# sabarim/STEm-Seg

Measured on AMD Instinct MI355X. Metric: clips/sec (T=8, 480p) embed+cluster, higher is better.
Workload: dtype f16x3: fp32 emulated from 2 fp16 terms per operand (22-bit operand significands; fp32 has 24), power-of-two operand scaling, 3 fp16 MFMA products per fp32 product, fp32 accumulate; |activation| >= 2.6e5 -> non-finite, flagged on the device, clip re-run in bf16x6

## Files before the change

### include/stemseg_hip.h

```cpp
#ifndef STEMSEG_HIP_H
#define STEMSEG_HIP_H

#include <stddef.h>
#include <stdint.h>

#ifdef __cplusplus
extern "C" {
#endif

#define STEMSEG_HIP_ABI_VERSION 11

#define STEMSEG_OK              0
#define STEMSEG_E_INVALID      -1
#define STEMSEG_E_HIP          -2
#define STEMSEG_E_WORKSPACE    -3
#define STEMSEG_E_UNSUPPORTED  -4

#define STEMSEG_MAX_HEAD_OUT   10
#define STEMSEG_MAX_WIDE_HEAD_OUT 64
#define STEMSEG_MAX_INSTANCES  64
#define STEMSEG_MAX_EMB_DIMS    8
#define STEMSEG_MAX_SEMSEG_CLASSES 128

int         stemseg_hip_version(void);
const char* stemseg_hip_last_error(void);
int         stemseg_hip_device_count(void);

int stemseg_hip_profile_enable(int32_t on);
int stemseg_hip_profile_read(double* out_host, int32_t n_tags);

typedef struct StemsegVolume {
    float*  ptr;
    int64_t c_stride, t_stride, y_stride;
    int32_t C, T, H, W;
    int64_t limit;
} StemsegVolume;

int stemseg_hip_padded_geometry(int32_t C, int32_t T, int32_t H, int32_t W, int64_t out[5]);


int stemseg_hip_pack_conv_weight(const float* w, float* packed, int32_t Cout, int32_t Cin, int32_t taps, void* stream);

#define STEMSEG_TILE_CFG_DEEP 8
typedef struct StemsegConvEpilogue {
    int32_t      relu;
    const float* residual;
    int64_t      res_c_stride, res_t_stride, res_y_stride;
    int32_t      decode_H, decode_W;
    int32_t      precision;
    int32_t      frames, plan_frames;
    int64_t      plan_scratch_floats;
} StemsegConvEpilogue;
#define STEMSEG_PRECISION_F32    0
#define STEMSEG_PRECISION_BF16X6 2
#define STEMSEG_PRECISION_F16X3  3
int64_t stemseg_hip_packed_weight_bytes_prec(int32_t Cout, int32_t Cin, int32_t taps, int32_t precision);
int stemseg_hip_pack_conv_weight_prec(const float* w, void* packed, int32_t Cout, int32_t Cin, int32_t taps, int32_t precision, void* stream);
int stemseg_hip_conv3d(const StemsegVolume* in, const float* packed_w, const float* bias, const StemsegVolume* out,
                       int32_t kt, int32_t kh, int32_t kw, int32_t tile_cfg, float* splitk_scratch,
                       int64_t splitk_scratch_floats, const StemsegConvEpilogue* epilogue, void* stream);
int stemseg_hip_conv3d_zero_t_halo(const StemsegVolume* in, const float* packed_w, const float* bias, const StemsegVolume* out,
                                   int32_t kt, int32_t kh, int32_t kw, int32_t tile_cfg, float* splitk_scratch,
                                   int64_t splitk_scratch_floats, const StemsegConvEpilogue* epilogue, int32_t groups, float eps,
                                   float* stats, double* gn_scratch, void* stream);
int stemseg_hip_conv3d_zero_t_halo_clips(const StemsegVolume* in, const float* packed_w, const float* bias, const StemsegVolume* out,
                                         int32_t kt, int32_t kh, int32_t kw, int32_t tile_cfg, float* splitk_scratch,
                                         int64_t splitk_scratch_floats, const StemsegConvEpilogue* epilogue, int32_t groups, float eps,
                                         float* stats, double* gn_scratch, int32_t plan_clips, void* stream);

int stemseg_hip_conv3d_zero_t_halo_batch(const StemsegVolume* in, const float* packed_w, const float* bias, const StemsegVolume* out,
                                         int32_t kt, int32_t kh, int32_t kw, int32_t tile_cfg, const StemsegConvEpilogue* epilogue,
                                         int32_t n_clips, int64_t in_clip_stride, int64_t out_clip_stride, void* stream);

typedef struct StemsegConvPlanRecord {
    int32_t kt, kh, kw;
    int32_t ck, mt;
    int32_t rows, tw, nt;
    int32_t flat, pmax;
    int32_t gl, blk;
    int32_t threads;
    int32_t precision;
    int32_t ksplit, chunks_per_split, nchunks;
    int32_t grid[3];
    int32_t row0, row1;
    int32_t vec4, vec_epi;
    int32_t reduce;
    int32_t gn;
    int32_t zero_t_halo;
    int32_t nb;
    int32_t deep;
} StemsegConvPlanRecord;
#define STEMSEG_PLAN_GN          1
#define STEMSEG_PLAN_ZERO_T_HALO 2
int stemseg_hip_conv3d_plan(const StemsegVolume* in, const float* bias, const StemsegVolume* out, int32_t kt, int32_t kh, int32_t kw,
                            int32_t tile_cfg, const float* splitk_scratch, int64_t splitk_scratch_floats,
                            const StemsegConvEpilogue* epilogue, int32_t form, int32_t gn_groups, StemsegConvPlanRecord* records,
                            int32_t capacity, int32_t* count);
int stemseg_hip_conv3d_plan_clips(const StemsegVolume* in, const float* bias, const StemsegVolume* out, int32_t kt, int32_t kh, int32_t kw,
                                  int32_t tile_cfg, const float* splitk_scratch, int64_t splitk_scratch_floats,
                                  const StemsegConvEpilogue* epilogue, int32_t form, int32_t gn_groups, int32_t plan_clips,
                                  StemsegConvPlanRecord* records, int32_t capacity, int32_t* count);

int64_t stemseg_hip_packed_grouped_weight_bytes(int32_t Cout, int32_t Cin_g, int32_t groups, int32_t precision);
int stemseg_hip_pack_grouped_conv_weight(const float* w, void* packed, int32_t Cout, int32_t Cin_g, int32_t groups, int32_t precision, void* stream);
int stemseg_hip_conv2d_grouped(const StemsegVolume* in, const void* packed_w, const float* bias, const StemsegVolume* out, int32_t groups,
                               int32_t stride, int32_t relu, int32_t precision, int32_t plan_frames, void* stream);

int64_t stemseg_hip_conv3d_gn_scratch_doubles(int32_t Cout, int32_t groups);
int stemseg_hip_conv3d_gn(const StemsegVolume* in, const float* packed_w, const float* bias, const StemsegVolume* out,
                          int32_t kt, int32_t kh, int32_t kw, int32_t tile_cfg, float* splitk_scratch,
                          int64_t splitk_scratch_floats, int32_t precision, int32_t groups, float eps,
                          float* stats, double* gn_scratch, void* stream);

int stemseg_hip_groupnorm_stats(const float* x, int32_t C, int64_t S, int32_t groups, float eps,
                                float* stats, double* scratch, void* stream);

int stemseg_hip_gn_relu_pool(const float* x, int32_t C, int32_t T, int32_t H, int32_t W, int32_t groups,
                             const float* stats, const float* gamma, const float* beta, int32_t pool,
                             const StemsegVolume* out, void* stream);

int stemseg_hip_upsample_trilinear(const float* in, int32_t C, int32_t T, int32_t H, int32_t W,
                                   int32_t st, int32_t sy, int32_t sx, const StemsegVolume* out, void* stream);

int stemseg_hip_copy_to_volume(const float* in, int32_t layout, const StemsegVolume* out, void* stream);

// ... 448 lines not shown
```

### stem-seg_amd/csrc/bottleneck_fused.hip

```cpp
#include "common.h"
#include "split_operand.h"

namespace stemseg {

typedef float f32x16 __attribute__((ext_vector_type(16)));
typedef _Float16 f16x8 __attribute__((ext_vector_type(8)));
typedef unsigned int u32x4 __attribute__((ext_vector_type(4)));

struct FusedTailParams {
    const unsigned int* x16;
    const char* w3;
    const float* b3;
    const float* res;
    float* y;
    const char* w1;
    const float* b1;
    float* z;
    int64_t z_cs, z_ts, z_ys;
    int dec_H, dec_W;
    int V;
    const float* xs;
    const char* wd;
    const float* bd;
    float* xsub;
    int sub_V;
};

constexpr SplitLayout FT_WL = SplitLayout(1, STEMSEG_PRECISION_F16X3);
static_assert(FT_WL.CK == 32 && FT_WL.G == 2 && FT_WL.NPL == 2, "the fused tail walks 32-channel chunks of two k-groups, two planes");

template <bool LAT>
__device__ __forceinline__ float slot_act(const float v) { return LAT ? v : relu_keep_nan(v); }

template <int MID_, int CT_, int P_, int DS_ = 0, int N1_ = MID_, bool LAT_ = false>
struct FusedTailCfg {
    static constexpr int MID = MID_, CT = CT_, COUT = 4 * MID_;
    static constexpr int N1 = N1_;
    static constexpr bool LAT = LAT_;
    static constexpr int DS = DS_, NCD = DS_ / 32;
    static constexpr int P = P_, NW = P_ / 32, NTHREADS = 64 * NW;
    static constexpr int NC3 = MID / 32;
    static constexpr int NCT = COUT / CT;
    static constexpr int MI3 = CT / 32, MI1 = N1 / 32;
    static constexpr int NH = 2 * MI3;
    static constexpr int UNROLL3 = LAT && NC3 <= 2 ? NC3 : 1;
    static constexpr int X_BYTES = 2 * 4 * P * 16;
    static constexpr int W3_BYTES = 8 * CT * 16;
    static constexpr int W1_HALF = 4 * N1 * 16;
    static constexpr int LDS_BYTES = 2 * X_BYTES + 2 * W3_BYTES + 2 * W1_HALF;
    static constexpr int NQ = P / 64;
    static constexpr int X_PIECES = X_BYTES / 1024, W3_PIECES = W3_BYTES / 1024, W1_PIECES = W1_HALF / 1024;
    static_assert(NC3 == FT_WL.chunks(MID) && W3_BYTES == FT_WL.slab_bytes(CT, 32) && W1_HALF * FT_WL.G == FT_WL.slab_bytes(N1, 32), "tile byte sizes follow the packed-weight layout");
    static_assert(P % 64 == 0 && MID % 32 == 0 && N1 % 32 == 0 && CT % 32 == 0 && COUT % CT == 0 && 2 * N1 * 4 <= 2 * X_BYTES, "tile shapes");
    static_assert(LDS_BYTES <= (P <= 128 ? 80 : 160) * 1024, "LDS: two 128-position workgroups, or one 256-position workgroup, per CU");
    static_assert(W3_BYTES % 1024 == 0 && W1_HALF % 1024 == 0 && X_PIECES % NW == 0, "whole DMA pieces");
    static_assert(MI1 * 16 + MI3 * 16 + (DS ? MI3 * 16 : 0) <= 176, "accumulators must leave room for fragments at 256 registers");
    static_assert(DS % 32 == 0 && 2 * CT * 4 <= W1_HALF, "shortcut: whole K-chunks; its (1 / scale, bias) table waits in a w1 buffer");
};

template <class C>
__global__ __launch_bounds__(C::NTHREADS, 2) void fused_tail_kernel(const FusedTailParams p) {
#pragma clang fp contract(off)
    __shared__ __attribute__((aligned(1024))) char smem[C::LDS_BYTES];
    char* const xbuf = smem;
    char* const w3buf = smem + 2 * C::X_BYTES;
    char* const w1buf = smem + 2 * C::X_BYTES + 2 * C::W3_BYTES;

    const int tid = threadIdx.x, lane = tid & 63;
    const int wave = __builtin_amdgcn_readfirstlane(tid >> 6);
    const int half = lane >> 5, l31 = lane & 31;
    const int pos0 = blockIdx.x * C::P;
    const int pos = pos0 + wave * 32 + l31;
    const bool pos_ok = pos < p.V;
    const int pos_c = min(pos, p.V - 1);
    const int64_t V = p.V;
    const unsigned int lane_off = (unsigned int)(((int64_t)(4 * half) * V + pos_c) * 4);
    auto opaque = [](unsigned int v) __attribute__((always_inline)) { asm volatile("" : "+v"(v)); return v; };
    const unsigned int SV4 = C::LAT ? (unsigned int)p.sub_V * 4u : 0u;
// ... 245 lines not shown
                        __builtin_amdgcn_raw_buffer_store_b32(__builtin_bit_cast(unsigned int, v0), rsub, sub_off, (row + 0) * SV4, 0);
                        __builtin_amdgcn_raw_buffer_store_b32(__builtin_bit_cast(unsigned int, v1), rsub, sub_off, (row + 1) * SV4, 0);
                        __builtin_amdgcn_raw_buffer_store_b32(__builtin_bit_cast(unsigned int, v2), rsub, sub_off, (row + 2) * SV4, 0);
                        __builtin_amdgcn_raw_buffer_store_b32(__builtin_bit_cast(unsigned int, v3), rsub, sub_off, (row + 3) * SV4, 0);
                    }
                    split_pair_f16(v0, v1, hw[2 * q], lw[2 * q]);
                    split_pair_f16(v2, v3, hw[2 * q + 1], lw[2 * q + 1]);
                }
                __builtin_amdgcn_sched_barrier(0);
#pragma unroll
                for (int gg = 0; gg < 2; ++gg) {
                    unsigned int xh[2], yh[2], xl[2], yl[2];
#pragma unroll
                    for (int i = 0; i < 2; ++i) {
                        auto sh = __builtin_amdgcn_permlane32_swap(hw[4 * gg + i], hw[4 * gg + 2 + i], false, false);
                        xh[i] = sh[0]; yh[i] = sh[1];
                        auto sl = __builtin_amdgcn_permlane32_swap(lw[4 * gg + i], lw[4 * gg + 2 + i], false, false);
                        xl[i] = sl[0]; yl[i] = sl[1];
                    }
                    const u32x4 bh = {xh[0], xh[1], yh[0], yh[1]}, bl = {xl[0], xl[1], yl[0], yl[1]};
                    b_hi[gg] = __builtin_bit_cast(f16x8, bh);
                    b_lo[gg] = __builtin_bit_cast(f16x8, bl);
                }
            } else if (m + 1 < C::MI3) {
                if constexpr (!DSV) load_identity(co_j + (m + 1) * 32, rres);
            }
            __builtin_amdgcn_sched_barrier(0);
            if (h + 1 < C::NH) dma_w1(j, h + 1, (h + 1) & 1);
            else if (j + 1 < C::NCT) {
                if constexpr (DSV) { dma_wd(j + 1, 0, sb); load_xs(xr); }
                else { dma_x(0, sb); dma_w3(j + 1, 0, sb); }
            } else dma_tail_tab();
            const char* w1b = w1buf + (h & 1) * C::W1_HALF + (half * C::N1 + l31) * 16;
            f16x8 a_hi[2], a_lo[2];
            auto ld_a1 = [&](const int m1, const int k) __attribute__((always_inline)) {
                a_hi[k] = *reinterpret_cast<const f16x8*>(w1b + ((0 * 2) * C::N1 + m1 * 32) * 16);
                a_lo[k] = *reinterpret_cast<const f16x8*>(w1b + ((1 * 2) * C::N1 + m1 * 32) * 16);
            };
            ld_a1(0, 0);
#pragma unroll
            for (int m1 = 0; m1 < C::MI1; ++m1) {
                if (m1 + 1 < C::MI1) ld_a1(m1 + 1, (m1 + 1) & 1);
                __builtin_amdgcn_sched_barrier(0);
                mma3(acc1[m1], a_hi[m1 & 1], a_lo[m1 & 1], b_hi[g], b_lo[g]);
                __builtin_amdgcn_sched_barrier(0);
            }
            stage_sync();
        }
    }
    if (pos_ok) {
        const int hwp = p.dec_H * p.dec_W;
        const int t2 = pos / hwp, r2 = pos - t2 * hwp, y2 = r2 / p.dec_W, x2 = r2 - y2 * p.dec_W;
        const unsigned int z_off = (unsigned int)(((int64_t)(4 * half) * p.z_cs + (int64_t)t2 * p.z_ts + (int64_t)y2 * p.z_ys + x2) * 4);
#pragma unroll
        for (int m1 = 0; m1 < C::MI1; ++m1)
#pragma unroll
            for (int q = 0; q < 4; ++q) {
                const int co4 = m1 * 32 + 8 * q + 4 * half;
                const float4 sc = *reinterpret_cast<const float4*>(reinterpret_cast<const float*>(xbuf) + co4);
                const float4 bv = *reinterpret_cast<const float4*>(reinterpret_cast<const float*>(xbuf) + C::N1 + co4);
                char* zo = reinterpret_cast<char*>(p.z + (int64_t)(m1 * 32 + 8 * q) * p.z_cs);
                *reinterpret_cast<float*>(zo + (size_t)z_off) = slot_act<C::LAT>(__fadd_rn(__fmul_rn(acc1[m1][4 * q + 0], sc.x), bv.x));
                *reinterpret_cast<float*>(zo + p.z_cs * 4 + (size_t)z_off) = slot_act<C::LAT>(__fadd_rn(__fmul_rn(acc1[m1][4 * q + 1], sc.y), bv.y));
                *reinterpret_cast<float*>(zo + p.z_cs * 8 + (size_t)z_off) = slot_act<C::LAT>(__fadd_rn(__fmul_rn(acc1[m1][4 * q + 2], sc.z), bv.z));
                *reinterpret_cast<float*>(zo + p.z_cs * 12 + (size_t)z_off) = slot_act<C::LAT>(__fadd_rn(__fmul_rn(acc1[m1][4 * q + 3], sc.w), bv.w));
            }
    }
}


typedef float f32x4 __attribute__((ext_vector_type(4)));

template <int MID_>
struct FusedTail16Cfg {
    static constexpr int MID = MID_, COUT = 4 * MID_, CT = 128;
    static constexpr int NW = 8, NTHREADS = 512, P = 16 * NW;
    static constexpr int NC3 = MID / 32, NCT = COUT / CT;
    static constexpr int NT3 = CT / 16, NT1 = MID / 16;
    static constexpr int SC = 2;
    static constexpr int NS = NC3 / SC, NU = CT / 32;
    static constexpr int W3_CHUNK = 8 * CT * 16;
    static constexpr int W3_BYTES = SC * W3_CHUNK;
    static constexpr int W1_BYTES = 8 * MID * 16;
    static constexpr int TAB_BYTES = 2 * CT * 4;
    static constexpr int LDS_BYTES = 2 * W3_BYTES + 2 * W1_BYTES + 2 * TAB_BYTES;
    static_assert(NC3 % SC == 0 && W3_BYTES % (1024 * NW) == 0 && W1_BYTES % (1024 * NW) == 0 && TAB_BYTES == 1024, "whole DMA pieces per wave");
    static_assert(W3_CHUNK == FT_WL.slab_bytes(CT, FT_WL.CK) && W1_BYTES == FT_WL.slab_bytes(MID, FT_WL.CK), "tile byte sizes follow the packed-weight layout");
    static_assert(LDS_BYTES <= 160 * 1024 && 2 * MID * 4 <= W3_BYTES, "LDS");
};

template <class C>
__global__ __launch_bounds__(C::NTHREADS, 2) void fused_tail16_kernel(const FusedTailParams p) {
#pragma clang fp contract(off)
    __shared__ __attribute__((aligned(1024))) char smem[C::LDS_BYTES];
    char* const w3buf = smem;
    char* const w1buf = smem + 2 * C::W3_BYTES;
    char* const tabbuf = smem + 2 * C::W3_BYTES + 2 * C::W1_BYTES;

    const int tid = threadIdx.x, lane = tid & 63;
    const int wave = __builtin_amdgcn_readfirstlane(tid >> 6);
    const int n = lane & 15, kb = lane >> 4;
    const int pos = blockIdx.x * C::P + wave * 16 + n;
    const bool pos_ok = pos < p.V;
    const int pos_c = min(pos, p.V - 1);
    const int64_t V = p.V;
    const unsigned int lane_off = (unsigned int)(((int64_t)(4 * kb) * V + pos_c) * 4);
    auto opaque = [](unsigned int v) __attribute__((always_inline)) { asm volatile("" : "+v"(v)); return v; };
    typedef const __attribute__((address_space(1))) void* gptr_t;
    typedef __attribute__((address_space(3))) void* lptr_t;
    const float* inv3 = reinterpret_cast<const float*>(p.w3 + FT_WL.inv_offset(C::COUT, C::MID));
    const float* inv1 = reinterpret_cast<const float*>(p.w1 + FT_WL.inv_offset(C::MID, C::COUT));

    auto dma_w3 = [&](const int j, const int st, const int buf) __attribute__((always_inline)) {
        constexpr int PER_ROW = C::CT * 16 / 1024, PER_CHUNK = C::W3_CHUNK / 1024;
#pragma unroll
        for (int k = 0; k < C::W3_BYTES / 1024 / C::NW; ++k) {
            const int idx = wave + k * C::NW, sc = idx / PER_CHUNK, r = idx % PER_CHUNK, row = r / PER_ROW, part = r % PER_ROW;
            const char* src = p.w3 + ((int64_t)(st * C::SC + sc) * 8 + row) * (C::COUT * 16) + (int64_t)j * (C::CT * 16) + part * 1024 + (size_t)(opaque((unsigned int)lane) * 16u);
// ... 524 lines not shown
                    a_hi[k][e] = *reinterpret_cast<const f16x8*>(w1b + (((g * 2 + 0) * 2) * C::N1 + (2 * mp + e) * 32) * 16);
                    a_lo[k][e] = *reinterpret_cast<const f16x8*>(w1b + (((g * 2 + 1) * 2) * C::N1 + (2 * mp + e) * 32) * 16);
                }
            };
            ld1(0, 0);
            ld1(1, 1);
            a_his[0][0] = a_hi[0][0] * k2048;
            a_his[0][1] = a_hi[0][1] * k2048;
#pragma unroll
            for (int s = 0; s < C::NX1; ++s) {
                __builtin_amdgcn_sched_barrier(0);
                if (s < C::S0) {
#pragma unroll
                    for (int k = C::M_PPS * s; k < C::M_PPS * s + C::M_PPS; ++k) {
                        if (u + 1 < C::NU) { if (k < C::W1_PIECES) dma_w1(j * C::NU + u + 1, eb ^ 1, k); }
                        else if (j + 1 < C::NCT) { if constexpr (DSV) dma_wd(j + 1, 0, sb, k); else dma_w3(j + 1, 0, sb, k); }
                    }
                }
                if (!DSV && s == C::S0) load_identity(u + 2 < C::NU ? j : min(j + 1, C::NCT - 1), (u + 2) % C::NU, rres[u & 1]);
                if (s + 2 < C::NX1) ld1(s + 2, (s + 2) % 3);
                if (s + 1 < C::NX1) {
                    a_his[(s + 1) & 1][0] = a_hi[(s + 1) % 3][0] * k2048;
                    a_his[(s + 1) & 1][1] = a_hi[(s + 1) % 3][1] * k2048;
                }
                if (u + 1 < C::NU) {
                    constexpr int SE = C::S0 + 4 / C::SL;
                    if (s >= C::S0 && s < SE) {
#pragma unroll
                        for (int q = 0; q < C::SL; ++q) e_slice(u + 1, (s - C::S0) * C::SL + q);
                    }
                    if (C::SL == 1 ? s == SE : s == SE) e_perm(0, b_hi[(u + 1) & 1][0], b_lo[(u + 1) & 1][0]);
                    if (C::SL == 1 ? s == SE + 1 : s == SE) e_perm(1, b_hi[(u + 1) & 1][1], b_lo[(u + 1) & 1][1]);
                }
                const int g = s / (C::MI1 / 2), mp = s % (C::MI1 / 2);
                mma6(acc1[2 * mp], acc1[2 * mp + 1], a_hi[s % 3], a_lo[s % 3], a_his[s & 1], b_hi[u & 1][g], b_lo[u & 1][g]);
#pragma unroll
                for (int i = 0; i < 6; ++i) { FT_SGB(0x008, 1); FT_SGB(0x100, 1); FT_SGB(0x002, 7 * C::SL); FT_SGB(0x040, C::SL * (C::LAT ? 2 : 1)); FT_SGB(0x020, 3); }
            }
            __builtin_amdgcn_sched_barrier(0);
            if (u + 1 < C::NU) FT_VMCNT(DSV ? C::EST : 16 + C::EST);
            else FT_VMCNT(DSV ? 0 : 16);
            __syncthreads();
            eb ^= 1;
        }
    }
    static_assert(C::N1 / 4 <= 64, "one lane per four channels");
    if (wave < 2 && lane < C::N1 / 4)
        *reinterpret_cast<float4*>(w3buf + wave * (C::N1 * 4) + lane * 16) = *reinterpret_cast<const float4*>((wave == 0 ? inv1 : p.b1) + lane * 4);
    __syncthreads();
    if (pos_ok) {
        const int hwp = p.dec_H * p.dec_W;
        const int t2 = pos / hwp, r2 = pos - t2 * hwp, y2 = r2 / p.dec_W, x2 = r2 - y2 * p.dec_W;
        const unsigned int z_off = (unsigned int)(((int64_t)(4 * half) * p.z_cs + (int64_t)t2 * p.z_ts + (int64_t)y2 * p.z_ys + x2) * 4);
        const float* ttab = reinterpret_cast<const float*>(w3buf);
#pragma unroll
        for (int m1 = 0; m1 < C::MI1; ++m1)
#pragma unroll
            for (int q = 0; q < 4; ++q) {
                const int co4 = m1 * 32 + 8 * q + 4 * half;
                const float4 sc = *reinterpret_cast<const float4*>(ttab + co4);
                const float4 bv = *reinterpret_cast<const float4*>(ttab + C::N1 + co4);
                char* zo = reinterpret_cast<char*>(p.z + (int64_t)(m1 * 32 + 8 * q) * p.z_cs);
                *reinterpret_cast<float*>(zo + (size_t)z_off) = slot_act<C::LAT>(__fadd_rn(__fmul_rn(acc1[m1][4 * q + 0], sc.x), bv.x));
                *reinterpret_cast<float*>(zo + p.z_cs * 4 + (size_t)z_off) = slot_act<C::LAT>(__fadd_rn(__fmul_rn(acc1[m1][4 * q + 1], sc.y), bv.y));
                *reinterpret_cast<float*>(zo + p.z_cs * 8 + (size_t)z_off) = slot_act<C::LAT>(__fadd_rn(__fmul_rn(acc1[m1][4 * q + 2], sc.z), bv.z));
                *reinterpret_cast<float*>(zo + p.z_cs * 12 + (size_t)z_off) = slot_act<C::LAT>(__fadd_rn(__fmul_rn(acc1[m1][4 * q + 3], sc.w), bv.w));
            }
    }
}

template <class C>
static int launch_fused_r1_cfg(const FusedTailParams& p, hipStream_t s) {
    const double flops = 2.0 * 2.0 * (double)C::MID * C::COUT * (double)p.V;
    void* ev = profile_begin(19, flops, s);
    hipLaunchKernelGGL(fused_tail_r1_kernel<C>, dim3((unsigned)ceil_div(p.V, C::P)), dim3(C::NTHREADS), 0, s, p);
    profile_end(ev, s);
    SS_LAUNCH_CHECK();
    return STEMSEG_OK;
}

template <class C>
static int launch_fused16_cfg(const FusedTailParams& p, hipStream_t s) {
    const double flops = 2.0 * 2.0 * (double)C::MID * C::COUT * (double)p.V;
    void* ev = profile_begin(19, flops, s);
    hipLaunchKernelGGL(fused_tail16_kernel<C>, dim3((unsigned)ceil_div(p.V, C::P)), dim3(C::NTHREADS), 0, s, p);
    profile_end(ev, s);
    SS_LAUNCH_CHECK();
    return STEMSEG_OK;
}

template <class C>
static int launch_fused_cfg(const FusedTailParams& p, hipStream_t s) {
    const double flops = 2.0 * 2.0 * (double)C::MID * C::COUT * (double)p.V;
    void* ev = profile_begin(19, flops, s);
    hipLaunchKernelGGL(fused_tail_kernel<C>, dim3((unsigned)ceil_div(p.V, C::P)), dim3(C::NTHREADS), 0, s, p);
    profile_end(ev, s);
    SS_LAUNCH_CHECK();
    return STEMSEG_OK;
}

constexpr int FT_STAGE_END_TAG = 52;
template <class C, class K>
static int launch_stage_end_cfg(K kernel, const FusedTailParams& p, hipStream_t s) {
    const double flops = 2.0 * ((double)C::MID + C::N1) * C::COUT * (double)p.V;
    void* ev = profile_begin(FT_STAGE_END_TAG, flops, s);
    hipLaunchKernelGGL(kernel, dim3((unsigned)ceil_div(p.V, C::P)), dim3(C::NTHREADS), 0, s, p);
    profile_end(ev, s);
    SS_LAUNCH_CHECK();
    return STEMSEG_OK;
}

bool fused_tail_supported(int mid) { return mid == 64 || mid == 128 || mid == 256; }

bool fused_shortcut_supported(int mid, int cin, int64_t V) {
    return ((mid == 64 && cin == 64) || (mid == 128 && cin == 256)) && (int64_t)cin * V * 4 < (1ll << 32) - (1 << 20) && (int64_t)128 * V * 4 < (1ll << 32) - (1 << 20);
}

bool fused_stage_end_supported(int mid, int64_t V) {
    return (mid == 64 || mid == 128 || mid == 256) && V > 0 && V <= (1ll << 27) && (int64_t)128 * V * 4 < (1ll << 32) - (1 << 20);
}

int launch_fused_stage_end(int mid, const unsigned int* x16, const float* w3, const float* b3, const float* res, float* y, const float* wl, const float* bl,
                           float* lat, float* xsub, int T, int h, int w, hipStream_t s) {
    const int64_t V = (int64_t)T * h * w;
    SS_CHECK_ARG(x16 && w3 && b3 && res && y && wl && bl && lat && xsub, "fused_stage_end: null pointer");
    SS_CHECK_ARG(T > 0 && h > 0 && w > 0 && h % 2 == 0 && w % 2 == 0 && fused_stage_end_supported(mid, V), "fused_stage_end: mid = %d, %d planes of %d x %d (even)", mid, T, h, w);
    SS_CHECK_ARG(reinterpret_cast<uintptr_t>(x16) % 16 == 0 && reinterpret_cast<uintptr_t>(w3) % 16 == 0 && reinterpret_cast<uintptr_t>(wl) % 16 == 0 &&
                 reinterpret_cast<uintptr_t>(b3) % 16 == 0 && reinterpret_cast<uintptr_t>(bl) % 16 == 0, "fused_stage_end: 16-byte aligned operands");
    FusedTailParams p;
    p.x16 = x16; p.w3 = reinterpret_cast<const char*>(w3); p.b3 = b3; p.res = res; p.y = y;
    p.w1 = reinterpret_cast<const char*>(wl); p.b1 = bl;
    p.z = lat; p.z_cs = V; p.z_ts = (int64_t)h * w; p.z_ys = w; p.dec_H = h; p.dec_W = w;
    p.V = (int)V;
    p.xs = nullptr; p.wd = nullptr; p.bd = nullptr;
    p.xsub = xsub; p.sub_V = (int)((int64_t)T * (h / 2) * (w / 2));
    if (mid == 256) { using C = FusedTailR1Cfg<256, 128, 0, 256, true>; return launch_stage_end_cfg<C>(fused_tail_r1_kernel<C>, p, s); }
    if (mid == 128) { using C = FusedTailR1Cfg<128, 128, 0, 256, true>; return launch_stage_end_cfg<C>(fused_tail_r1_kernel<C>, p, s); }
    using C = FusedTailCfg<64, 64, 128, 0, 256, true>;
    return launch_stage_end_cfg<C>(fused_tail_kernel<C>, p, s);
}

int launch_fused_tail(int mid, const unsigned int* x16, const float* w3, const float* b3, const float* res, float* y, const float* w1, const float* b1,
                      const StemsegVolume& z, int dec_H, int dec_W, int64_t V, int form, hipStream_t s, const float* ds_x, int ds_cin, const float* ds_w,
                      const float* ds_b) {
    SS_CHECK_ARG(x16 && w3 && b3 && y && w1 && b1 && z.ptr, "fused_tail: null pointer");
    SS_CHECK_ARG(ds_x ? (!res && ds_w && ds_b && fused_shortcut_supported(mid, ds_cin, V) && reinterpret_cast<uintptr_t>(ds_w) % 16 == 0 && reinterpret_cast<uintptr_t>(ds_b) % 16 == 0)
                      : res != nullptr, "fused_tail: identity map, or a shortcut (mid %d, %d input channels) this library has a kernel for", mid, ds_cin);
    SS_CHECK_ARG(fused_tail_supported(mid), "fused_tail: mid = %d (64, 128 or 256)", mid);
    SS_CHECK_ARG(V > 0 && V <= (1ll << 27) && z.c_stride <= (1ll << 27) && dec_H > 0 && dec_W > 0 && V % ((int64_t)dec_H * dec_W) == 0, "fused_tail: V = %lld positions of %d x %d planes",
                 (long long)V, dec_H, dec_W);
    SS_CHECK_ARG(z.C == mid, "fused_tail: consumer volume has %d channels, conv1 makes %d", z.C, mid);
    SS_CHECK_ARG(reinterpret_cast<uintptr_t>(x16) % 16 == 0 && reinterpret_cast<uintptr_t>(w3) % 16 == 0 && reinterpret_cast<uintptr_t>(w1) % 16 == 0 &&
                 reinterpret_cast<uintptr_t>(b3) % 16 == 0 && reinterpret_cast<uintptr_t>(b1) % 16 == 0, "fused_tail: 16-byte aligned operands");
    FusedTailParams p;
    p.x16 = x16; p.w3 = reinterpret_cast<const char*>(w3); p.b3 = b3; p.res = res; p.y = y;
    p.w1 = reinterpret_cast<const char*>(w1); p.b1 = b1;
    p.z = z.ptr; p.z_cs = z.c_stride; p.z_ts = z.t_stride; p.z_ys = z.y_stride; p.dec_H = dec_H; p.dec_W = dec_W;
    p.V = (int)V;
    p.xs = ds_x; p.wd = reinterpret_cast<const char*>(ds_w); p.bd = ds_b;
    p.xsub = nullptr; p.sub_V = 0;
    if (ds_x && mid == 128) return launch_fused_r1_cfg<FusedTailR1Cfg<128, 128, 256>>(p, s);
    if (ds_x) return launch_fused_cfg<FusedTailCfg<64, 128, 128, 64>>(p, s);
    if (mid == 256) {
        const bool r1_fits = (int64_t)128 * V * 4 < (1ll << 32) - (1 << 20);
        if (form != 1 && r1_fits) return launch_fused_r1_cfg<FusedTailR1Cfg<256, 128>>(p, s);
        return launch_fused16_cfg<FusedTail16Cfg<256>>(p, s);
    }
    if (mid == 128 && form != 1 && (int64_t)128 * V * 4 < (1ll << 32) - (1 << 20)) return launch_fused_r1_cfg<FusedTailR1Cfg<128, 128>>(p, s);
    if (mid == 128) return launch_fused_cfg<FusedTailCfg<128, 128, 128>>(p, s);
    return launch_fused_cfg<FusedTailCfg<64, 128, 128>>(p, s);
}

}
```

### stem-seg_amd/csrc/common.h

```cpp
#pragma once
#include <hip/hip_runtime.h>
#include <cstdarg>
#include <cstdint>
#include <cstdio>
#include <cstring>

#include "../../include/stemseg_hip.h"

#if defined(__HIP_DEVICE_COMPILE__) && defined(__AMDGCN_WAVEFRONT_SIZE) && __AMDGCN_WAVEFRONT_SIZE != 64
#error "libstemseg_hip is written for 64-lane wavefronts (gfx950): shuffles, ballots and MFMA layouts assume it"
#endif

namespace stemseg {

void set_error(const char* fmt, ...);

#define SS_CHECK_ARG(cond, ...)                                     \
    do {                                                            \
        if (!(cond)) {                                              \
            ::stemseg::set_error(__VA_ARGS__);                      \
            return STEMSEG_E_INVALID;                               \
        }                                                           \
    } while (0)

// ... 53 lines not shown
    SS_CHECK_ARG(v.limit >= (int64_t)(v.C - 1) * v.c_stride + frame_end, "%s: the view %s reaches past its limit", who, name);
    return STEMSEG_OK;
}

struct BBView {
    const float* ptr;
    int64_t cs, ts, ys;
};

__device__ __forceinline__ float relu_mask(float y, float v) {
    const unsigned u = __float_as_uint(y), mag = u & 0x7fffffffu;
    const bool blocked = mag == 0u || ((u >> 31) != 0u && mag <= 0x7f800000u);
    return blocked ? 0.f : v;
}

constexpr int WS_GUARD_FLOATS = 64;
constexpr uint32_t WS_CANARY = 0x7fc5ca7au;
constexpr int WS_MAX_GUARDS = 64;
struct GuardList {
    int n = 0;
    int64_t off[WS_MAX_GUARDS];
    bool full = false;
    void push(int64_t o) { if (n < WS_MAX_GUARDS) off[n++] = o; else full = true; }
};
int launch_canary_fill(float* ws, const GuardList& g, hipStream_t s);
int canary_check(const float* ws, const GuardList& g, int32_t* n_bad_host, int64_t* first_bad_host, hipStream_t s);

void* profile_begin(int tag, double work, hipStream_t s);
void profile_end(void* handle, hipStream_t s);

struct PlanSink {
    StemsegConvPlanRecord* rec;
    int cap, n;
    int row0 = 0;
};

struct ConvEpilogue {
    int relu = 0;
    const float* res = nullptr;
    int64_t res_cs = 0, res_ts = 0, res_ys = 0;
    int dec_H = 0, dec_W = 0;
    int precision = 0;
    int frames = 0, plan_frames = 0;
    int64_t plan_scratch_floats = 0;
    double* gn_part = nullptr;
    int gn_cpg = 0, gn_cap = 0;
    int* gn_used = nullptr;
    int nb = 1;
    int64_t in_bs = 0, out_bs = 0, gn_bs = 0;
    int plan_clips = 0;
    unsigned int* p16_out = nullptr;
    int* p16_done = nullptr;
    int p16_keep_plan = 0;
    int zero_t_halo = 0;
    PlanSink* plan_sink = nullptr;
};
int launch_conv3d(const StemsegVolume& in, const float* packed_w, const float* bias, const StemsegVolume& out,
                  int kt, int kh, int kw, int tile_cfg, hipStream_t s, float* splitk_scratch = nullptr, int64_t splitk_scratch_floats = 0,
                  const ConvEpilogue* epi = nullptr);
int launch_grouped_conv(const StemsegVolume& in, const void* packed_w, const float* bias, const StemsegVolume& out, int groups, int stride,
                        int relu, int precision, hipStream_t s);
bool fused_tail_supported(int mid);
int launch_fused_tail(int mid, const unsigned int* x16, const float* w3, const float* b3, const float* res, float* y, const float* w1, const float* b1,
                      const StemsegVolume& z, int dec_H, int dec_W, int64_t V, int form, hipStream_t s, const float* ds_x = nullptr, int ds_cin = 0,
                      const float* ds_w = nullptr, const float* ds_b = nullptr);
bool fused_shortcut_supported(int mid, int cin, int64_t V);
int launch_gn_stats(const float* x, int C, int64_t S, int groups, float eps, float* stats, double* scratch, hipStream_t s);
bool fused_stage_end_supported(int mid, int64_t V);
int launch_fused_stage_end(int mid, const unsigned int* x16, const float* w3, const float* b3, const float* res, float* y, const float* wl, const float* bl,
                           float* lat, float* xsub, int T, int h, int w, hipStream_t s);
constexpr int GN_SLOT_CAP = 32768;
static inline int64_t gn_scratch_doubles(int Cout, int groups) { return (int64_t)groups * GN_SLOT_CAP * 2 > (int64_t)groups * 128 ? (int64_t)groups * GN_SLOT_CAP * 2 : (int64_t)groups * 128; }
int launch_conv3d_gn(const StemsegVolume& in, const float* packed_w, const float* bias, const StemsegVolume& out, int kt, int kh, int kw,
                     int tile_cfg, hipStream_t s, float* splitk_scratch, int64_t splitk_scratch_floats, const ConvEpilogue* epi, int groups,
                     float eps, float* stats, double* gn_scratch, int64_t stats_bs = 0);
int launch_gn_identity_stats(float* stats, int groups, hipStream_t s);
struct ClipBatch {
    int nb = 1;
    int64_t in_bs = 0, out_bs = 0, stats_bs = 0;
};
int launch_gn_finalize_slots(const double* part, int groups, int cap, int used, double group_elems, float eps, float* stats, hipStream_t s,
                             int nb = 1, int64_t part_bs = 0, int64_t stats_bs = 0);
int launch_gn_relu_pool(const float* x, int C, int T, int H, int W, int groups, const float* stats, const float* gamma,
                        const float* beta, int pool, const StemsegVolume& out, hipStream_t s, const ClipBatch& cb = ClipBatch());
int launch_upsample(const float* in, int C, int T, int H, int W, int st, int sy, int sx, const StemsegVolume& out,
                    hipStream_t s, const ClipBatch& cb = ClipBatch());
int launch_copy_to_volume(const float* in, int layout, const StemsegVolume& out, hipStream_t s);
int launch_copy_strided(const float* in, int64_t in_c_stride, int64_t in_t_stride, const StemsegVolume& out, hipStream_t s);
struct HeadSpec {
    int n_out;
    int act[STEMSEG_MAX_EMB_DIMS * 2];
    int grid_axis[STEMSEG_MAX_EMB_DIMS * 2];
};
struct HeadsGN {
    const float* stats;
    const float* gamma;
    const float* beta;
    int cpg;
    int64_t stats_bs;
};
int launch_heads(const float* x, int Cin, int T, int H, int W, const float* w, const float* bias, const HeadSpec& hs,
                 const float* gt, const float* gy, const float* gx, float* out, hipStream_t s, const ClipBatch& cb = ClipBatch(),
                 const float* add = nullptr, int64_t add_bs = 0, const HeadsGN* gn = nullptr);
int launch_level_head(const float* x, int Cin, int64_t V, const float* w, int n_out, const float* add, float* out, hipStream_t s, int nb, int64_t x_bs,
                      int64_t add_bs, int64_t out_bs);

}
```

### stem-seg_amd/csrc/conv_igemm.h

```cpp
#pragma once
#include "common.h"
#include "split_operand.h"
#include <algorithm>
#include <type_traits>

namespace stemseg {

typedef float f32x16 __attribute__((ext_vector_type(16)));

constexpr int MIN_WG4 = 4;

struct ConvKParams {
    const float* in;
    int64_t in_cs, in_ts, in_ys, in_limit;
    int in_H;
    const float* wpk;
    const float* bias;
    float* out;
    int64_t out_cs, out_ts, out_ys;
    int Cin, Cout, T, H, W;
    int tiles_x, tiles_y;
    int vec4;
    int chunks_per_split;
    int64_t out_split_stride;
    int relu;
    const float* res;
    int64_t res_cs, res_ts, res_ys;
    int dec_H, dec_W;
    int vec_epi;
    int t_fastest;
    int flat_t;
    int T_all;
    int n_co;
    double* gn_part;
    int gn_cpg, gn_cap, gn_slot0;
    int* gn_used_host;
    int nb;
    int zero_t_halo;
    int64_t in_bs, out_bs, gn_bs;
    unsigned int* out_p16;
};

template <int KT_, int KH_, int KW_, int CK_, int MI_, int NI_, int WM_, int WN_, int COLS_, bool PIPE_ = false, int BF_ = 0, bool DB_ = false,
          int PMAX_ = 0, bool GL_ = false, int BLK_ = 0>
struct ConvCfg {
    static constexpr bool PIPE = PIPE_, X6 = BF_ >= 2, F16 = BF_ == 3, DB = DB_, FLAT = PMAX_ > 0, GL = GL_;
    static_assert(BF_ == 0 || BF_ == 2 || BF_ == 3, "precision: 0 fp32-input MFMA, 2 bf16x6, 3 f16x3");
    static constexpr int NPX = BF_ == 2 ? 3 : 2;
    static constexpr int NPROD = BF_ == 2 ? 6 : 3;
    static constexpr int PMAX = PMAX_;
    static constexpr int KT = KT_, KH = KH_, KW = KW_, CK = CK_, MI = MI_, NI = NI_, WM = WM_, WN = WN_, COLS = COLS_;
    static constexpr int TAPS = KT * KH * KW;
    static constexpr int NTHREADS = 64 * WM * WN;
    static constexpr int MT = WM * MI * 32;
    static constexpr int NSEG = WN * NI;
    static constexpr bool BLK = BLK_ != 0;
    static constexpr bool DEEP = BLK_ < 0;
    static constexpr int TD = DEEP ? WN_ : 1;
    static constexpr int TPL = DEEP ? TD + 2 : KT_;
    static constexpr int NLIVE = (BLK && !DEEP) ? BLK_ * COLS_ : NSEG;
    static constexpr int ROWS = DEEP ? 4 * NI_ : (BLK ? 4 * BLK_ : NSEG / COLS);
    static constexpr int TW = BLK ? 8 * COLS_ : COLS_ * 32;
    static constexpr int RH = ROWS + KH - 1;
    static constexpr int XL = (TW + KW - 1 + 3) / 4;
    static constexpr int XP = DEEP ? 24 : (BLK ? ((4 * XL + 23) / 32) * 32 + 8 : 4 * XL);
    static constexpr int NT = NSEG * 32;
    static constexpr int FL = NT + 2 * PMAX + 8;
    static constexpr int IN_CH_STRIDE = FLAT ? KT * FL : KT * RH * XP;
    static constexpr int IN_PAIR_STRIDE = PMAX_ > 0 ? KT * (WN_ * NI_ * 32 + 2 * PMAX_ + 8) : TPL * RH * XP;
    static constexpr int IN_PLANE_STRIDE = (CK / 2) * IN_PAIR_STRIDE;
    static constexpr int IN_FLOATS = X6 ? NPX * IN_PLANE_STRIDE : CK * IN_CH_STRIDE;
    static constexpr SplitLayout SL = SplitLayout(TAPS, BF_, CK_);
    static_assert(BF_ < 2 || CK_ == split_chunk_channels(TAPS, BF_), "split-staged tiles walk the channel chunks the weights were packed in");
    static constexpr int TPG = SL.TPG, CPH = SL.CPH, NTG = SL.NTG;
    static constexpr int NCG = X6 ? SL.NCG : 1;
    static constexpr int G = NTG * NCG;
    static constexpr int NPL = SL.NPL;
    static constexpr int W_FLOATS = X6 ? NPL * G * 2 * MT * 4 : CK * TAPS * MT;
    static constexpr int GA = (G + 1) / 2;
    static constexpr int WMODE = (BF_ >= 2 && G <= 2) ? (BF_ == 3 ? 1 : ((WM * WN >= 8 || MI * NI < 8) ? 2 : 0)) : 0;
    static constexpr bool SP = WMODE == 1, LA = WMODE == 2;
    static constexpr int BUF_FLOATS = IN_FLOATS + W_FLOATS;
    static constexpr int LDS_FLOATS = BUF_FLOATS * (DB ? 2 : 1);
    static_assert(!X6 || CK % (2 * CPH) == 0, "split-staged: a chunk holds whole k-groups");
    static_assert(BLK || NSEG % COLS == 0, "segments must fill whole rows");
    static_assert(!BLK || (BF_ >= 2 && PMAX_ == 0 && NI_ == 2 && NLIVE <= NSEG && NLIVE > NSEG - NI_ && XP % 32 == (DEEP ? 24 : 8) && XP >= 4 * XL), "block tiles: split-staged, the last wave may lack its second block");
    static_assert(!DEEP || (BF_ == 3 && KT_ == 3 && WM_ == 1 && COLS_ == 1 && BLK_ == -1), "deep tile: f16x3, 3x3x3, one wave per output plane");
    static_assert(CK % 4 == 0 || (DB && GL_ && CK == 2 && !X6), "channel chunk is a multiple of the packed sub-chunk (4), or one channel pair (GL)");
    static_assert(LDS_FLOATS * 4 <= (X6 ? 160 : 80) * 1024, "two workgroups per CU (x6 eight-wave tiles: one)");
    static_assert(!X6 || (!DB && !GL && G >= 2 && CK % 2 == 0), "x6: 2-D / 3-D tiles, two weight phases");
    static_assert(!FLAT || (KH == 3 && KW == 3 && PMAX % 4 == 0), "flat tiles: 3x3 taps");
    static_assert(DB == GL_, "two LDS buffers are the direct-to-LDS form");
    static_assert(!GL || (DB && !X6), "direct-to-LDS staging is the double-buffered fp32 form");
    static constexpr int NWAVES = WM * WN;
    static constexpr int MIN_WG = X6 ? (MI * NI > 8 ? 1 : NWAVES >= 8 ? 2 : (LDS_FLOATS * 4 * 2 <= 160 * 1024 ? NWAVES / 2 : NWAVES / 4))
                                     : ((GL && LDS_FLOATS * 4 * 4 <= 140 * 1024 && MI * NI <= 4) ? MIN_WG4 : ((GL && LDS_FLOATS * 4 * 3 <= 160 * 1024) ? 3 : 2));
};

template <class C>
__global__ __launch_bounds__(C::NTHREADS, C::MIN_WG) void conv_igemm_kernel(const ConvKParams p) {
    __shared__ __attribute__((aligned(16))) float smem[C::LDS_FLOATS];
    float* const in_lds = smem;
    float* const w_lds = smem + C::IN_FLOATS;

    const int tid = threadIdx.x;
    const int lane = tid & 63;
    const int wave = __builtin_amdgcn_readfirstlane(tid >> 6);
    const int wm = wave / C::WN, wn = wave % C::WN;
    const int half = lane >> 5, l31 = lane & 31;

    int bx;
    {
        const int nwg = gridDim.x, xcd = blockIdx.x & 7, q = nwg >> 3, r = nwg & 7;
        bx = (xcd < r ? xcd * (q + 1) : r * (q + 1) + (xcd - r) * q) + (blockIdx.x >> 3);
    }
    const int co_tile = bx % p.n_co;
    bx /= p.n_co;
    int tx, ty, t;
    if constexpr (C::DEEP) {
        tx = bx % p.tiles_x;
        ty = bx / p.tiles_x;
        t = 0;
    } else if (C::KT > 1 && p.t_fastest) {
        t = bx % p.T;
        bx /= p.T;
        tx = bx % p.tiles_x;
        ty = bx / p.tiles_x;
    } else {
        tx = bx % p.tiles_x;
        bx /= p.tiles_x;
        ty = bx % p.tiles_y;
        t = bx / p.tiles_y;
    }
    const int x0 = C::FLAT ? 0 : tx * C::TW, y0 = C::FLAT ? 0 : ty * C::ROWS;
    constexpr bool TV = C::KT == 3 && C::X6 && !C::FLAT && (C::F16 || C::MI * C::NI < 8);
    int tvar = 0;
    if constexpr (TV) {
        if constexpr (C::DEEP) tvar = wn == 0 ? 1 : (wn == C::WN - 1 ? 2 : 0);
        else if (p.zero_t_halo && p.T > 1) tvar = t == 0 ? 1 : (t == p.T - 1 ? 2 : 0);
    }
    const int svar = C::DEEP ? 0 : tvar;
    const int t_out = C::DEEP ? wn : t;
    auto seg_row = [](const int sN, const int l) __attribute__((always_inline)) { return C::DEEP ? (sN % C::NI) * 4 + (l >> 3) : (C::BLK ? (sN / C::COLS) * 4 + (l >> 3) : sN / C::COLS); };
    auto seg_col = [](const int sN, const int l) __attribute__((always_inline)) { return C::DEEP ? (l & 7) : (C::BLK ? (sN % C::COLS) * 8 + (l & 7) : (sN % C::COLS) * 32 + l); };
    const bool ni1_live = !C::BLK || (wn * C::NI + 1 < C::NLIVE);
    const int pitch = (int)p.in_ys;
    const int F0 = pitch + tx * C::NT;
    const int co0 = co_tile * C::MT;

    f32x16 acc[C::MI][C::NI];
#pragma unroll
    for (int mi = 0; mi < C::MI; ++mi)
#pragma unroll
        for (int ni = 0; ni < C::NI; ++ni)
#pragma unroll
            for (int r = 0; r < 16; ++r) acc[mi][ni][r] = 0.f;

    const float* a_ptr = w_lds + half * C::MT + wm * (C::MI * 32) + l31;
    const float* b_ptr[C::NI];
#pragma unroll
    for (int ni = 0; ni < C::NI; ++ni) {
        const int s = wn * C::NI + ni;
        b_ptr[ni] = C::FLAT ? in_lds + half * C::IN_CH_STRIDE + s * 32 + l31 + 3
                            : in_lds + half * C::IN_CH_STRIDE + seg_row(s, l31) * C::XP + seg_col(s, l31);
    }

    const unsigned int* b_ptr6[C::NI];
#pragma unroll
    for (int ni = 0; ni < C::NI; ++ni) {
        const int s = wn * C::NI + ni;
        b_ptr6[ni] = C::FLAT ? reinterpret_cast<const unsigned int*>(in_lds) + half * (C::CPH / 2) * C::IN_PAIR_STRIDE + s * 32 + l31 + 3
                             : reinterpret_cast<const unsigned int*>(in_lds) + half * (C::CPH / 2) * C::IN_PAIR_STRIDE + seg_row(min(s, C::NLIVE - 1), l31) * C::XP + seg_col(min(s, C::NLIVE - 1), l31);
        if constexpr (C::DEEP) b_ptr6[ni] += wn * (C::RH * C::XP);
    }
    const float* in_tile = p.in + (int64_t)blockIdx.y * p.in_bs + (int64_t)t * p.in_ts + x0;
    const int64_t tile_base = (int64_t)t * p.in_ts + x0;

    constexpr int XQ = C::XP / 4;
    constexpr int NQ = C::FLAT ? C::IN_FLOATS / 4 : C::CK * C::KT * C::RH * XQ;
    constexpr int MQ = C::MT / 4;
    constexpr int NWQ = C::X6 ? C::NPL * C::G * 2 * C::MT : C::CK * C::TAPS * MQ;
    constexpr int IN_PT = (NQ + C::NTHREADS - 1) / C::NTHREADS, W_PT = (NWQ + C::NTHREADS - 1) / C::NTHREADS;
    auto fetch_in = [&](int c0, int q) -> float4 {
        if constexpr (C::FLAT) {
            constexpr int FQ = C::FL / 4;
            const int j4 = q % FQ, rr = q / FQ, dt = rr % C::KT, c = rr / C::KT;
            const int f = F0 - pitch - 4 + 4 * j4;
            const int64_t rel = (int64_t)(c0 + c) * p.in_cs + (int64_t)dt * p.in_ts + f;
            float4 v = make_float4(0.f, 0.f, 0.f, 0.f);
            if (c0 + c < p.Cin && f >= 0 && 4 * j4 < C::NT + 2 * pitch + 8 && tile_base + rel + 4 <= p.in_limit)
                v = *reinterpret_cast<const float4*>(in_tile + rel);
            return v;
        }
        const int xq = q % XQ;
        int rr = q / XQ;
        const int r = rr % C::RH;
        rr /= C::RH;
        const int dt = rr % C::KT;
        const int c = rr / C::KT;
        const int yy = min(y0 + r, p.in_H - 1);
        const int64_t rel = (int64_t)(c0 + c) * p.in_cs + (int64_t)dt * p.in_ts + (int64_t)yy * p.in_ys + xq * 4;
        float4 v = make_float4(0.f, 0.f, 0.f, 0.f);
        if (c0 + c < p.Cin && tile_base + rel + 4 <= p.in_limit) v = *reinterpret_cast<const float4*>(in_tile + rel);
        return v;
    };
    auto fetch_w = [&](int c0, int q) -> float4 {
        const int mq = q % MQ;
        if constexpr (C::CK == 2) {
            const int row2 = q / MQ, tap = row2 >> 1, e = row2 & 1;
            const float* wsrc2 = p.wpk + ((int64_t)(c0 / 4) * (C::TAPS * 4) + tap * 4 + ((c0 >> 1) & 1) * 2 + e) * p.Cout + co0;
            float4 v2 = make_float4(0.f, 0.f, 0.f, 0.f);
            if (c0 + e < p.Cin && co0 + mq * 4 < p.Cout) v2 = *reinterpret_cast<const float4*>(wsrc2 + mq * 4);
            return v2;
        }
        const int row = q / MQ;
        const int ch = c0 + (row / (C::TAPS * 4)) * 4 + (row & 3);
        const float* wsrc = p.wpk + (int64_t)(c0 / 4) * (C::TAPS * 4) * p.Cout + co0;
        float4 v = make_float4(0.f, 0.f, 0.f, 0.f);
        if (ch < p.Cin && co0 + mq * 4 < p.Cout) v = *reinterpret_cast<const float4*>(wsrc + (int64_t)row * p.Cout + mq * 4);
        return v;
    };
    auto addr_in = [&](int c0, int q) -> const float* {
        int64_t rel;
        if constexpr (C::FLAT) {
            constexpr int FQ = C::FL / 4;
            const int j4 = q % FQ, rr = q / FQ, dt = rr % C::KT, c = rr / C::KT;
            const int f = max(F0 - pitch - 4 + 4 * j4, 0);
            rel = (int64_t)(c0 + c) * p.in_cs + (int64_t)dt * p.in_ts + f;
// ... 55 lines not shown
        }
        for (int q = tid; q < NWQ; q += C::NTHREADS) *reinterpret_cast<float4*>(w_lds + q * 4) = fetch_w(c0, q);
    };

    auto split3 = [](const float x, unsigned int& h, unsigned int& m, unsigned int& l) {
        unsigned short sh, sm, sl = 0;
        if constexpr (C::F16) split_act_f16(x, sh, sm);
        else split_bf16x3(x, sh, sm, sl);
        h = sh; m = sm; l = sl;
    };
    constexpr int FQ6 = C::FL / 4;
    constexpr int XL6 = C::XL;
    constexpr int NQ6 = C::FLAT ? (C::CK / 2) * C::KT * FQ6 : (C::CK / 2) * (C::DEEP ? C::TD : C::KT) * C::RH * XL6;
    auto in6_lds = [](const int q) __attribute__((always_inline)) {
        if constexpr (C::DEEP) return (q / XL6 + (q / (XL6 * C::RH * C::TD)) * 2 * C::RH + C::RH) * C::XP + (q % XL6) * 4;
        else return C::BLK ? (q / XL6) * C::XP + (q % XL6) * 4 : q * 4;
    };
    constexpr int IN_PT6 = C::X6 ? (NQ6 + C::NTHREADS - 1) / C::NTHREADS : 1;
    constexpr int NWQ_A = C::NPL * C::GA * 2 * C::MT, NWQ6 = C::NPL * C::G * 2 * C::MT;
    auto in6_rel = [&](int q, int& c) -> int64_t {
        if constexpr (C::FLAT) {
            const int j4 = q % FQ6, rr = q / FQ6, dt = rr % C::KT;
            c = 2 * (rr / C::KT);
            const int f = F0 - pitch - 4 + 4 * j4;
            if (f < 0 || 4 * j4 >= C::NT + 2 * pitch + 8) return -1;
            return (int64_t)c * p.in_cs + (int64_t)dt * p.in_ts + f;
        }
        const int xq = q % XL6;
        int rr = q / XL6;
        const int r = rr % C::RH;
        rr /= C::RH;
        constexpr int NPLQ = C::DEEP ? C::TD : C::KT;
        const int dt = rr % NPLQ + (C::DEEP ? 1 : 0);
        c = 2 * (rr / NPLQ);
        const int yy = min(y0 + r, p.in_H - 1);
        return (int64_t)c * p.in_cs + (int64_t)dt * p.in_ts + (int64_t)yy * p.in_ys + xq * 4;
    };
    auto fetch_in6 = [&](int c0, int q, float4& v0, float4& v1) {
        int c;
        const int64_t rel0 = in6_rel(q, c);
        const int64_t rel = rel0 + (int64_t)c0 * p.in_cs;
        v0 = v1 = make_float4(0.f, 0.f, 0.f, 0.f);
        if (rel0 < 0) return;
        if (c0 + c < p.Cin && tile_base + rel + 4 <= p.in_limit) v0 = *reinterpret_cast<const float4*>(in_tile + rel);
        if (c0 + c + 1 < p.Cin && tile_base + rel + p.in_cs + 4 <= p.in_limit) v1 = *reinterpret_cast<const float4*>(in_tile + rel + p.in_cs);
    };
    unsigned int in6_voff[IN_PT6];
    int in6_clim[IN_PT6];
    const int64_t in6_room = (p.in_limit - 4 - tile_base) * 4;
    constexpr int R6 = C::RH * XL6;
    constexpr int NQ6V = TV ? (C::CK / 2) * 2 * R6 : NQ6;
    constexpr int IN_PT6V = TV ? (NQ6V + C::NTHREADS - 1) / C::NTHREADS : IN_PT6;
    auto in6_live = [](const int qv, const int first) __attribute__((always_inline)) { return qv + (qv / (2 * R6)) * R6 + (first ? R6 : 0); };
    if constexpr (C::X6) {
#pragma unroll
        for (int k = 0; k < IN_PT6; ++k) {
            int q = tid + k * C::NTHREADS;
            bool inside = q < NQ6;
            if constexpr (TV && !C::DEEP) {
                if (tvar) { inside = q < NQ6V; q = inside ? in6_live(q, tvar == 1) : 0; }
            }
            int c = 0;
            const int64_t rel0 = inside ? in6_rel(q, c) : 0;
            const int64_t rel = rel0 < 0 ? 0 : rel0;
            in6_voff[k] = (unsigned int)(rel * 4);
            const int64_t slack = in6_room - rel * 4;
            const int64_t by_room = slack < 0 ? 0 : slack / (p.in_cs * 4) + 1;
            in6_clim[k] = (inside && rel0 >= 0) ? (int)min((int64_t)(p.Cin - c), by_room) : 0;
        }
    }
    typedef float f32x4 __attribute__((ext_vector_type(4)));
    auto fetch_in6_fast = [&](int c0, int k, f32x4& v0, f32x4& v1) __attribute__((always_inline)) {
        const char* base = reinterpret_cast<const char*>(in_tile) + (int64_t)c0 * p.in_cs * 4;
        const unsigned int cs4 = (unsigned int)(p.in_cs * 4);
        v0 = *reinterpret_cast<const f32x4*>(base + (c0 < in6_clim[k] ? in6_voff[k] : 0u));
        v1 = *reinterpret_cast<const f32x4*>(base + (c0 + 1 < in6_clim[k] ? in6_voff[k] + cs4 : 0u));
    };
    auto store_in6 = [&](int q, const float4& v0, const float4& v1) {
        unsigned int h0, m0, l0, h1, m1, l1;
        uint4 ph, pm, pl;
        if constexpr (C::F16) {
            split_pair_f16(v0.x, v1.x, ph.x, pm.x); split_pair_f16(v0.y, v1.y, ph.y, pm.y);
            split_pair_f16(v0.z, v1.z, ph.z, pm.z); split_pair_f16(v0.w, v1.w, ph.w, pm.w);
            unsigned int* d16 = reinterpret_cast<unsigned int*>(in_lds) + in6_lds(q);
            *reinterpret_cast<uint4*>(d16) = ph;
            *reinterpret_cast<uint4*>(d16 + C::IN_PLANE_STRIDE) = pm;
            return;
        }
        split3(v0.x, h0, m0, l0); split3(v1.x, h1, m1, l1); ph.x = h0 | (h1 << 16); pm.x = m0 | (m1 << 16); pl.x = l0 | (l1 << 16);
        split3(v0.y, h0, m0, l0); split3(v1.y, h1, m1, l1); ph.y = h0 | (h1 << 16); pm.y = m0 | (m1 << 16); pl.y = l0 | (l1 << 16);
        split3(v0.z, h0, m0, l0); split3(v1.z, h1, m1, l1); ph.z = h0 | (h1 << 16); pm.z = m0 | (m1 << 16); pl.z = l0 | (l1 << 16);
        split3(v0.w, h0, m0, l0); split3(v1.w, h1, m1, l1); ph.w = h0 | (h1 << 16); pm.w = m0 | (m1 << 16); pl.w = l0 | (l1 << 16);
        unsigned int* d = reinterpret_cast<unsigned int*>(in_lds) + in6_lds(q);
        *reinterpret_cast<uint4*>(d) = ph;
        *reinterpret_cast<uint4*>(d + C::IN_PLANE_STRIDE) = pm;
        if constexpr (C::NPX == 3) *reinterpret_cast<uint4*>(d + 2 * C::IN_PLANE_STRIDE) = pl;
    };
    auto store_in6_masked = [&](int c0, int k, int q, const f32x4& r0, const f32x4& r1) __attribute__((always_inline)) {
        const bool ok0 = c0 < in6_clim[k], ok1 = c0 + 1 < in6_clim[k];
        float4 v0, v1;
        v0.x = ok0 ? r0.x : 0.f; v0.y = ok0 ? r0.y : 0.f; v0.z = ok0 ? r0.z : 0.f; v0.w = ok0 ? r0.w : 0.f;
        v1.x = ok1 ? r1.x : 0.f; v1.y = ok1 ? r1.y : 0.f; v1.z = ok1 ? r1.z : 0.f; v1.w = ok1 ? r1.w : 0.f;
        store_in6(q, v0, v1);
    };
    auto stage_in6_direct = [&](int c0) {
        if (p.vec4) {
            for (int q = tid; q < NQ6; q += C::NTHREADS) {
                float4 v0, v1;
                fetch_in6(c0, q, v0, v1);
                store_in6(q, v0, v1);
            }
        } else if constexpr (!C::FLAT && !C::DEEP) {
            constexpr int NE6 = (C::CK / 2) * C::KT * C::RH * C::XP;
            for (int q = tid; q < NE6; q += C::NTHREADS) {
                const int xx = q % C::XP;
                int rr = q / C::XP;
                const int r = rr % C::RH;
                rr /= C::RH;
                const int dt = rr % C::KT;
                const int c = 2 * (rr / C::KT);
                const int yy = min(y0 + r, p.in_H - 1);
                const int64_t rel = (int64_t)(c0 + c) * p.in_cs + (int64_t)dt * p.in_ts + (int64_t)yy * p.in_ys + xx;
                float a0 = 0.f, a1 = 0.f;
                if (c0 + c < p.Cin && tile_base + rel < p.in_limit) a0 = in_tile[rel];
                if (c0 + c + 1 < p.Cin && tile_base + rel + p.in_cs < p.in_limit) a1 = in_tile[rel + p.in_cs];
                unsigned int h0, m0, l0, h1, m1, l1;
                split3(a0, h0, m0, l0);
                split3(a1, h1, m1, l1);
                unsigned int* d = reinterpret_cast<unsigned int*>(in_lds) + q;
                d[0] = h0 | (h1 << 16);
                d[C::IN_PLANE_STRIDE] = m0 | (m1 << 16);
                if constexpr (C::NPX == 3) d[2 * C::IN_PLANE_STRIDE] = l0 | (l1 << 16);
            }
        }
    };
    constexpr int W_PT6 = C::X6 ? ((C::SP ? NWQ6 : NWQ_A) + C::NTHREADS - 1) / C::NTHREADS : 1;
    static_assert(C::NTHREADS % C::MT == 0 && NWQ_A % C::MT == 0, "weight pieces: a thread keeps its column");
    const unsigned int w6_voff = C::X6 ? ((unsigned int)(tid / C::MT) * (unsigned int)p.Cout + (unsigned int)min(tid % C::MT, p.Cout - 1 - co0)) * 16u : 0u;
    auto w6_src = [&](int c0, int q_uniform) __attribute__((always_inline)) -> const char* {
        const char* base = reinterpret_cast<const char*>(p.wpk) +
                           (((int64_t)(c0 / C::CK) * (C::NPL * C::G * 2) + q_uniform / C::MT) * p.Cout + co0) * 16;
        return base + w6_voff;
    };
    auto compute6 = [&](auto g0c, auto g1c, auto&& side, auto live_c) __attribute__((always_inline)) {
        constexpr int g0 = decltype(g0c)::value, g1 = decltype(g1c)::value;
        constexpr bool LIVE1 = decltype(live_c)::value;
        constexpr int NPL = C::NPL, NPX = C::NPX, NA = 3;
        typedef typename std::conditional<C::F16, _Float16, __bf16>::type h16;
        typedef h16 h16x8 __attribute__((ext_vector_type(8)));
        const char* a_base = reinterpret_cast<const char*>(w_lds) + (half * C::MT + wm * (C::MI * 32) + l31) * 16;
        const unsigned int* bdy6[C::NI][3];
        if constexpr (C::FLAT) {
#pragma unroll
            for (int ni = 0; ni < C::NI; ++ni) { bdy6[ni][0] = b_ptr6[ni]; bdy6[ni][1] = b_ptr6[ni] + pitch; bdy6[ni][2] = b_ptr6[ni] + 2 * pitch; }
        }
        auto ld_b = [&](const int grp, h16x8 (&b)[NPX][C::NI]) __attribute__((always_inline)) {
            const int cg = grp / C::NTG, tg = grp % C::NTG;
#pragma unroll
            for (int ni = 0; ni < (LIVE1 ? C::NI : 1); ++ni)
#pragma unroll
                for (int pl = 0; pl < NPX; ++pl) {
                    uint4 w4;
                    unsigned int* wv = reinterpret_cast<unsigned int*>(&w4);
#pragma unroll
                    for (int wd = 0; wd < 4; ++wd) {
                        const int j0 = 2 * wd, tapi = j0 / C::CPH, chl = j0 % C::CPH;
                        int tap = tg * C::TPG + tapi;
                        tap = tap < C::TAPS ? tap : C::TAPS - 1;
                        const int dt = tap / (C::KH * C::KW), dy = (tap / C::KW) % C::KH, dx = tap % C::KW;
                        if constexpr (C::FLAT) {
                            const int off = pl * C::IN_PLANE_STRIDE + (cg * C::CPH + chl / 2) * C::IN_PAIR_STRIDE + dt * C::FL + dx;
                            wv[wd] = bdy6[ni][dy][off];
                        } else {
                            const int off = pl * C::IN_PLANE_STRIDE + (cg * C::CPH + chl / 2) * C::IN_PAIR_STRIDE + (dt * C::RH + dy) * C::XP + dx;
                            wv[wd] = b_ptr6[ni][off];
                        }
                    }
                    b[pl][ni] = __builtin_bit_cast(h16x8, w4);
                }
        };
        auto ld_a = [&](const int grp, const int mi, h16x8 (&a)[NA]) __attribute__((always_inline)) {
#pragma unroll
            for (int pl = 0; pl < NPL; ++pl)
                a[pl] = *reinterpret_cast<const h16x8*>(a_base + (((grp * NPL + pl) * 2) * C::MT + mi * 32) * 16);
        };
        auto mm = [&](const int mi, h16x8 (&a)[NA], const h16x8 (&b)[NPX][C::NI]) __attribute__((always_inline)) {
            if constexpr (C::F16) {
                a[2] = a[0] * (h16)(1.0f / F16X3_LO_SCALE);
#define SS_X6_TERM(PA, PB)                                                                                                     \
    _Pragma("unroll") for (int ni = 0; ni < (LIVE1 ? C::NI : 1); ++ni)                                                         \
        acc[mi][ni] = __builtin_amdgcn_mfma_f32_32x32x16_f16(a[PA], b[PB][ni], acc[mi][ni], 0, 0, 0);
                SS_X6_TERM(1, 0) SS_X6_TERM(2, 1) SS_X6_TERM(0, 0)
#undef SS_X6_TERM
            } else {
#define SS_X6_TERM(PA, PB)                                                                                                     \
    _Pragma("unroll") for (int ni = 0; ni < (LIVE1 ? C::NI : 1); ++ni)                                                         \
        acc[mi][ni] = __builtin_amdgcn_mfma_f32_32x32x16_bf16(a[PA], b[PB][ni], acc[mi][ni], 0, 0, 0);
                SS_X6_TERM(2, 0) SS_X6_TERM(0, 2) SS_X6_TERM(1, 1) SS_X6_TERM(1, 0) SS_X6_TERM(0, 1) SS_X6_TERM(0, 0)
#undef SS_X6_TERM
            }
        };
        constexpr int NSTEP = (g1 - g0) * C::MI;
        h16x8 bfr[NPX][C::NI], a0[NA], a1[NA];
        side(-1);
        ld_b(g0, bfr);
        ld_a(g0, 0, a0);
#pragma unroll
        for (int st = 0; st < NSTEP; st += 2) {
            const int mi = st % C::MI;
            if (st + 1 < NSTEP) ld_a(g0 + (st + 1) / C::MI, (st + 1) % C::MI, a1);
            side(st);
            __builtin_amdgcn_sched_barrier(0);
            mm(mi, a0, bfr);
            __builtin_amdgcn_sched_barrier(0);
// ... 716 lines not shown
```

### stem-seg_amd/csrc/conv_igemm.hip

```cpp
#include "conv_igemm.h"

namespace stemseg {

template <bool VEC>
__global__ __launch_bounds__(256) void splitk_reduce_kernel(const SplitReduceParams p) {
    constexpr int VW = VEC ? 4 : 1;
    const unsigned wq = (unsigned)p.W / VW;
    const unsigned c = blockIdx.y;
    const unsigned j = blockIdx.x * 256u + threadIdx.x;
    const bool active = j < p.per_c;
    const float* const partial = p.partial + (int64_t)blockIdx.z * p.part_bs;
    float* const outp = p.out + (int64_t)blockIdx.z * p.out_bs;
    float s1 = 0.f, s2 = 0.f;
    if (active) {
        const unsigned r2 = j / wq, x = (j - r2 * wq) * VW;
        const unsigned t = r2 / (unsigned)p.H, y = r2 - t * (unsigned)p.H;
        const int64_t i = (int64_t)c * p.V + (int64_t)r2 * p.W + x;
        const int64_t o = (int64_t)c * p.out_cs + (int64_t)t * p.out_ts + (int64_t)y * p.out_ys + x;
        if constexpr (VEC) {
            float4 acc = *reinterpret_cast<const float4*>(partial + i);
            for (int z = 1; z < p.ksplit; ++z) {
                const float4 v = *reinterpret_cast<const float4*>(partial + (int64_t)z * p.slab + i);
                acc.x += v.x; acc.y += v.y; acc.z += v.z; acc.w += v.w;
            }
// ... 66 lines not shown
    if (!p.vec4 || tile_cfg > 0 || p.dec_W > 0 || p.in_ys > Flat::PMAX || p.in_ys % 4 != 0 || p.W + 2 > p.in_ys) return false;
    return flat_tile_efficiency<Flat>(p) > 1.08 * tile_efficiency<Tile2D>(p.H, p.W);
}

template <class GLCfg, class Cfg>
static int launch_gl(const ConvKParams& p, const LaunchCtx& L) {
    if (p.vec4 && p.Cin % GLCfg::CK == 0 && p.Cout % GLCfg::MT == 0) return launch_cfg<GLCfg>(p, L);
    return launch_cfg<Cfg>(p, L);
}

int launch_conv3d(const StemsegVolume& in, const float* packed_w, const float* bias, const StemsegVolume& out,
                  int kt, int kh, int kw, int tile_cfg, hipStream_t s, float* scratch, int64_t scratch_floats, const ConvEpilogue* epi) {
    SS_CHECK_ARG(in.ptr && out.ptr && packed_w, "conv3d: null pointer");
    const bool deep_tile = tile_cfg == STEMSEG_TILE_CFG_DEEP;
    if (deep_tile) tile_cfg = 0;
    const int prec = epi ? epi->precision : STEMSEG_PRECISION_F32;
    SS_CHECK_ARG(prec == STEMSEG_PRECISION_F32 || prec == STEMSEG_PRECISION_BF16X6 || prec == STEMSEG_PRECISION_F16X3,
                 "conv3d: precision %d (0 f32, 2 bf16x6, 3 f16x3)", prec);
    const bool k3 = (kt == 3 && kh == 3 && kw == 3), k1 = (kt == 1 && kh == 1 && kw == 1), k2 = (kt == 1 && kh == 3 && kw == 3);
    const bool k4 = (kt == 1 && kh == 4 && kw == 4);
    SS_CHECK_ARG(k3 || k1 || k2 || (k4 && prec == STEMSEG_PRECISION_F16X3), "conv3d: kernel %dx%dx%d unsupported (3x3x3, 1x3x3, 1x1x1; 1x4x4 in f16x3 mode)", kt, kh, kw);
    const bool flat = epi && epi->dec_W > 0;
    if (flat) {
        SS_CHECK_ARG(k1 && in.T == 1 && in.H == 1 && epi->dec_H > 0 && (int64_t)out.T * out.H * out.W == in.W &&
                     out.H == epi->dec_H && out.W == epi->dec_W, "conv3d: flat-decode epilogue needs a 1x1x1 conv on a [C][V] input with V == T*H*W of `out`");
    } else {
        SS_CHECK_ARG(in.T == out.T + kt - 1 && in.H == out.H + kh - 1 && in.W == out.W + kw - 1,
                     "conv3d: input extents (%d,%d,%d) must be output (%d,%d,%d) + kernel - 1", in.T, in.H, in.W, out.T, out.H, out.W);
    }
    SS_CHECK_ARG(in.C % 4 == 0 && out.C % 32 == 0, "conv3d: Cin %% 4 == 0 and Cout %% 32 == 0 required (got %d, %d)", in.C, out.C);
    ConvKParams p;
    p.in = in.ptr; p.in_cs = in.c_stride; p.in_ts = in.t_stride; p.in_ys = in.y_stride; p.in_limit = in.limit; p.in_H = in.H;
    p.wpk = packed_w; p.bias = bias;
    p.out = out.ptr; p.out_cs = out.c_stride; p.out_ts = out.t_stride; p.out_ys = out.y_stride;
    p.Cin = in.C; p.Cout = out.C; p.T = out.T; p.H = out.H; p.W = out.W;
    if (flat) { p.T = 1; p.H = 1; p.W = in.W; }
    p.relu = epi ? epi->relu : 0;
    p.res = epi ? epi->res : nullptr;
    p.res_cs = epi ? epi->res_cs : 0; p.res_ts = epi ? epi->res_ts : 0; p.res_ys = epi ? epi->res_ys : 0;
    p.dec_H = flat ? epi->dec_H : 0; p.dec_W = flat ? epi->dec_W : 0;
    p.gn_part = epi ? epi->gn_part : nullptr;
    p.gn_cpg = epi ? epi->gn_cpg : 0; p.gn_cap = epi ? epi->gn_cap : 0; p.gn_slot0 = 0;
    p.gn_used_host = epi ? epi->gn_used : nullptr;
    p.zero_t_halo = (epi && epi->zero_t_halo && k3) ? 1 : 0;
    p.out_p16 = nullptr;
    if (epi && epi->p16_out) {
        const bool dense = out.t_stride == (int64_t)out.H * out.W && out.y_stride == out.W && out.c_stride == (int64_t)out.T * out.H * out.W;
        SS_CHECK_ARG(epi->p16_done && dense && !flat && !epi->res && !epi->gn_part && out.C % 8 == 0 && prec == STEMSEG_PRECISION_F16X3 && (!epi || epi->nb <= 1),
                     "conv3d: the pair-plane output needs f16x3, a dense output volume, no residual / statistics / clip batch");
        *epi->p16_done = 0;
        p.out_p16 = epi->p16_out;
        p.gn_used_host = epi->p16_done;
    }
    p.nb = (epi && epi->nb > 1) ? epi->nb : 1;
    p.in_bs = p.nb > 1 ? epi->in_bs : 0; p.out_bs = p.nb > 1 ? epi->out_bs : 0; p.gn_bs = p.nb > 1 ? epi->gn_bs : 0;
    SS_CHECK_ARG(p.nb == 1 || (!p.res && p.nb <= 65535 && p.in_bs % 4 == 0 && p.out_bs % 4 == 0), "conv3d: a clip batch takes no residual and 16-byte aligned clip strides");
    SS_CHECK_ARG(!p.gn_part || ((p.gn_cpg == 4 || p.gn_cpg == 8) && p.gn_used_host && p.Cout % p.gn_cpg == 0 && !(epi->relu || epi->res)),
                 "conv3d: fused GroupNorm statistics need groups of 4 or 8 channels and a plain (bias-only) epilogue");
    auto al16 = [](const void* ptr, int64_t cs, int64_t ts, int64_t ys, int T, int H) {
        return (reinterpret_cast<uintptr_t>(ptr) % 16 == 0) && (cs % 4 == 0) && (T == 1 || ts % 4 == 0) && (H == 1 || ys % 4 == 0);
    };
    p.vec_epi = (!flat && p.W % 4 == 0 && al16(p.out, p.out_cs, p.out_ts, p.out_ys, p.T, p.H) &&
                 (!p.res || al16(p.res, p.res_cs, p.res_ts, p.res_ys, p.T, p.H))) ? 1 : 0;
    p.tiles_x = p.tiles_y = 0;
    p.t_fastest = 1;
    p.flat_t = 0; p.T_all = p.T;
    const bool aligned = (reinterpret_cast<uintptr_t>(in.ptr) % 16 == 0) && (in.c_stride % 4 == 0) &&
                         (in.T == 1 || in.t_stride % 4 == 0) && (in.H == 1 || in.y_stride % 4 == 0);
    p.vec4 = aligned ? 1 : 0;
    SS_CHECK_ARG(reinterpret_cast<uintptr_t>(packed_w) % 16 == 0, "conv3d: packed weights must be 16-byte aligned");
    PlanCtx pc_store;
    const PlanCtx* pc = nullptr;
    if (epi && epi->plan_frames > 0) {
        SS_CHECK_ARG(epi->frames > 0 && epi->plan_scratch_floats >= 0, "conv3d: plan_frames needs the launch's own frame count");
        pc_store.shape = p;
        pc_store.scratch_floats = epi->plan_scratch_floats;
        if (p.T == 1 && p.H == 1) {
            SS_CHECK_ARG(p.W % epi->frames == 0, "conv3d: flat volume of %d voxels is not %d whole frames", p.W, epi->frames);
            const int64_t Wp = (int64_t)(p.W / epi->frames) * epi->plan_frames;
            SS_CHECK_ARG(Wp < (1ll << 31), "conv3d: planning volume too large");
            pc_store.shape.W = (int)Wp;
        } else {
            SS_CHECK_ARG(p.T == epi->frames, "conv3d: launch of %d t-planes announced as %d frames", p.T, epi->frames);
            pc_store.shape.T = epi->plan_frames;
        }
        pc_store.shape.T_all = pc_store.shape.T;
        pc = &pc_store;
    }
    const ConvKParams& d = pc ? pc->shape : p;
    SS_CHECK_ARG(!epi || (epi->plan_clips >= 0 && epi->plan_clips <= 4096), "conv3d: plan_clips %d", epi ? epi->plan_clips : 0);
    const LaunchCtx L{s, scratch, scratch_floats, pc, epi && epi->p16_keep_plan, epi ? epi->plan_sink : nullptr, epi && epi->plan_clips > 1 ? epi->plan_clips : 1, deep_tile};
    if (k4) return launch_stem_f16x3(p, L);
    if (prec == STEMSEG_PRECISION_BF16X6) return launch_split_family<2>(p, d, L, tile_cfg, k3, k2);
    if (prec == STEMSEG_PRECISION_F16X3) return launch_split_family<3>(p, d, L, tile_cfg, k3, k2);
    const bool auto_cfg = tile_cfg <= 0 || tile_cfg > 3;
    if (k3) {
        int cfg = tile_cfg;
        if (auto_cfg) {
            if (tile_workgroups<K3Big>(d) >= 512) cfg = 1;
            else if (tile_workgroups<K3Med>(d) >= 384) cfg = 2;
            else cfg = 3;
        }
        if (cfg == 2 && prefer_flat<K3FlatMed56, K3Med>(p, tile_cfg)) return launch_cfg<K3FlatMed56>(p, L);
        if (cfg == 3 && prefer_flat<K3FlatSmall56, K3Small>(p, tile_cfg)) return launch_cfg<K3FlatSmall56>(p, L);
        if (cfg == 2 && prefer_flat<K3FlatMed, K3Med>(p, tile_cfg)) return launch_cfg<K3FlatMed>(p, L);
        if (cfg == 3 && prefer_flat<K3FlatSmall, K3Small>(p, tile_cfg)) return launch_cfg<K3FlatSmall>(p, L);
// ... 135 lines not shown
extern "C" int stemseg_hip_conv3d_zero_t_halo_batch(const StemsegVolume* in, const float* packed_w, const float* bias, const StemsegVolume* out,
                                                    int32_t kt, int32_t kh, int32_t kw, int32_t tile_cfg, const StemsegConvEpilogue* epilogue,
                                                    int32_t n_clips, int64_t in_clip_stride, int64_t out_clip_stride, void* stream) {
    using namespace stemseg;
    SS_CHECK_ARG(in && out, "conv3d_zero_t_halo_batch: null volume");
    SS_CHECK_ARG(kt == 3, "conv3d_zero_t_halo: the promise is about the temporal halo planes of a kernel with kt == 3 (got %d)", kt);
    SS_CHECK_ARG(n_clips >= 1 && n_clips <= 4096 && in_clip_stride >= 0 && out_clip_stride >= 0, "conv3d_zero_t_halo_batch: n_clips=%d", n_clips);
    ConvEpilogue e = epilogue_from_abi(epilogue);
    e.zero_t_halo = 1;
    e.nb = n_clips; e.in_bs = in_clip_stride; e.out_bs = out_clip_stride;
    return launch_conv3d(*in, packed_w, bias, *out, kt, kh, kw, tile_cfg, as_stream(stream), nullptr, 0, &e);
}

static int conv3d_plan(const StemsegVolume* in, const float* bias, const StemsegVolume* out, int32_t kt, int32_t kh, int32_t kw, int32_t tile_cfg,
                       const float* splitk_scratch, int64_t splitk_scratch_floats, const StemsegConvEpilogue* epilogue, int32_t form,
                       int32_t gn_groups, int32_t plan_clips, StemsegConvPlanRecord* records, int32_t capacity, int32_t* count) {
    using namespace stemseg;
    SS_CHECK_ARG(in && out && count && capacity >= 0 && (records || capacity == 0), "conv3d_plan: null volume / record array");
    SS_CHECK_ARG((form & ~(STEMSEG_PLAN_GN | STEMSEG_PLAN_ZERO_T_HALO)) == 0, "conv3d_plan: form %d", form);
    alignas(16) static float no_weights[4];
    alignas(16) static double no_table[2];
    PlanSink sink{records, capacity, 0};
    ConvEpilogue e;
    const bool gn = (form & STEMSEG_PLAN_GN) != 0, zth = (form & STEMSEG_PLAN_ZERO_T_HALO) != 0;
    if (gn && !zth) e.precision = epilogue ? epilogue->precision : STEMSEG_PRECISION_F32;
    else e = epilogue_from_abi(epilogue);
    if (zth) {
        SS_CHECK_ARG(kt == 3, "conv3d_zero_t_halo: the promise is about the temporal halo planes of a kernel with kt == 3 (got %d)", kt);
        e.zero_t_halo = 1;
    }
    e.plan_sink = &sink;
    e.plan_clips = plan_clips;
    float* const scratch = const_cast<float*>(splitk_scratch);
    const int rc = gn ? launch_conv3d_gn(*in, no_weights, bias, *out, kt, kh, kw, tile_cfg, nullptr, scratch, splitk_scratch_floats, &e, gn_groups, 1e-5f,
                                         no_weights, no_table)
                      : launch_conv3d(*in, no_weights, bias, *out, kt, kh, kw, tile_cfg, nullptr, scratch, splitk_scratch_floats, &e);
    *count = sink.n;
    return rc;
}

extern "C" int stemseg_hip_conv3d_plan(const StemsegVolume* in, const float* bias, const StemsegVolume* out, int32_t kt, int32_t kh, int32_t kw,
                                       int32_t tile_cfg, const float* splitk_scratch, int64_t splitk_scratch_floats,
                                       const StemsegConvEpilogue* epilogue, int32_t form, int32_t gn_groups, StemsegConvPlanRecord* records,
                                       int32_t capacity, int32_t* count) {
    return conv3d_plan(in, bias, out, kt, kh, kw, tile_cfg, splitk_scratch, splitk_scratch_floats, epilogue, form, gn_groups, 0, records, capacity, count);
}

extern "C" int stemseg_hip_conv3d_plan_clips(const StemsegVolume* in, const float* bias, const StemsegVolume* out, int32_t kt, int32_t kh, int32_t kw,
                                             int32_t tile_cfg, const float* splitk_scratch, int64_t splitk_scratch_floats,
                                             const StemsegConvEpilogue* epilogue, int32_t form, int32_t gn_groups, int32_t plan_clips,
                                             StemsegConvPlanRecord* records, int32_t capacity, int32_t* count) {
    return conv3d_plan(in, bias, out, kt, kh, kw, tile_cfg, splitk_scratch, splitk_scratch_floats, epilogue, form, gn_groups, plan_clips, records, capacity, count);
}
```

### stem-seg_amd/csrc/conv_split_family.h

```cpp
#pragma once
#include "conv_igemm.h"

namespace stemseg {

template <int BFV>
struct SplitTiles {
    static constexpr int CK2 = split_chunk_channels(9, BFV);
    using Y3Big = ConvCfg<3, 3, 3, 4, 4, 2, 1, 8, 1, false, BFV>;
    using Y3Med = ConvCfg<3, 3, 3, 4, 2, 2, 2, 4, 1, false, BFV>;
    using Y3Small = ConvCfg<3, 3, 3, 4, 2, 1, 2, 4, 1, false, BFV>;
    using Y2Big = ConvCfg<1, 3, 3, CK2, 4, 2, 1, 8, 1, false, BFV>;
    using Y2Med = ConvCfg<1, 3, 3, CK2, 2, 2, 2, 2, 1, false, BFV>;
    using Y2Small = ConvCfg<1, 3, 3, CK2, 2, 1, 2, 2, 1, false, BFV>;
    using Y2M64 = ConvCfg<1, 3, 3, CK2, 2, 2, 1, 4, 1, false, BFV>;
    using Y1Big = ConvCfg<1, 1, 1, 32, 4, 2, 1, 4, 8, false, BFV>;
    using Y1Small = ConvCfg<1, 1, 1, 32, 2, 2, 2, 2, 4, false, BFV>;
    using Y1M64 = ConvCfg<1, 1, 1, 32, 2, 2, 1, 4, 8, false, BFV>;
    using Y1Wide = ConvCfg<1, 1, 1, 32, 4, 2, 2, 4, 8, false, BFV>;
    template <int PMAX> using Y2Flat = ConvCfg<1, 3, 3, CK2, 4, 2, 1, 8, 16, false, BFV, false, PMAX>;
    using Y4Stem = ConvCfg<1, 4, 4, 16, 2, 2, 1, 8, 1, false, BFV>;
    using Y3Blk = ConvCfg<3, 3, 3, 4, 4, 2, 1, 8, 3, false, BFV, false, 0, false, 5>;
    using Y2Blk = ConvCfg<1, 3, 3, CK2, 4, 2, 1, 8, 3, false, BFV, false, 0, false, 5>;
    using Y3Blk7 = ConvCfg<3, 3, 3, 4, 2, 2, 2, 4, 7, false, BFV, false, 0, false, 1>;
};

struct DeepTiles {
    using Y3Deep = ConvCfg<3, 3, 3, 4, 4, 2, 1, 8, 1, false, 3, false, 0, false, -1>;
};
template <class Deep>
static bool deep_tile_eligible(const ConvKParams& p, const ConvKParams& d, const LaunchCtx& L, bool k3) {
    if (!L.deep_tile || !k3 || !p.zero_t_halo || p.T != Deep::TD || d.T != Deep::TD || p.H % Deep::ROWS != 0 || p.W % Deep::TW != 0 || !p.vec4 || p.out_p16 || p.dec_W > 0) return false;
    ConvKParams q = p;
    q.T_all = q.T;
    return plan_ksplit<Deep>(q, L, 0, (int)ceil_div(p.Cin, Deep::CK)) == 1;
}

template <int BFV>
int launch_split_family(ConvKParams& p, const ConvKParams& d, const LaunchCtx& L, int tile_cfg, bool k3, bool k2) {
    float* const scratch = L.scratch;
    typedef SplitTiles<BFV> F;
    using Y3Big = typename F::Y3Big; using Y3Med = typename F::Y3Med; using Y3Small = typename F::Y3Small;
    using Y2Big = typename F::Y2Big; using Y2Med = typename F::Y2Med; using Y2Small = typename F::Y2Small; using Y2M64 = typename F::Y2M64;
    using Y1Small = typename F::Y1Small; using Y1Big = typename F::Y1Big; using Y1M64 = typename F::Y1M64; using Y1Wide = typename F::Y1Wide;
    const bool auto_cfg = tile_cfg <= 0 || tile_cfg > 3;
    int cfg = (auto_cfg || tile_cfg == 6) ? 0 : tile_cfg;
    if constexpr (BFV == 3) {
        const bool flat_ok = p.vec4 && p.dec_W == 0 && p.in_ys % 4 == 0 && p.W + 2 <= p.in_ys && p.in_ys <= 224 && p.Cout % 128 == 0;
        if (flat_ok && k2 && !p.gn_part && p.in_ts == (int64_t)p.in_H * p.in_ys && p.in_H == p.H + 2 &&
            (tile_cfg == 5 || (auto_cfg && tile_workgroups<Y2Big>(d) >= (scratch ? 96 : 384)))) {
            const double e2d = tile_efficiency<Y2Big>(p.H, p.W);
            const double efl = (double)d.T * p.H * p.W / (512.0 * ceil_div((int64_t)d.T * p.in_ts, 512));
            if (tile_cfg == 5 || (efl > 1.04 * e2d && p.in_ys <= 56)) {
                p.flat_t = 1;
                if (p.in_ys <= 56) return launch_cfg<typename F::template Y2Flat<56>>(p, L);
                if (p.in_ys <= 112) return launch_cfg<typename F::template Y2Flat<112>>(p, L);
                return launch_cfg<typename F::template Y2Flat<224>>(p, L);
            }
        }
    }
    if constexpr (BFV == 3) {
        if (deep_tile_eligible<DeepTiles::Y3Deep>(p, d, L, k3)) return launch_cfg<DeepTiles::Y3Deep>(p, L);
    }
    static_assert(F::Y2Blk::ROWS == F::Y3Blk::ROWS && F::Y2Blk::TW == F::Y3Blk::TW && Y2Big::ROWS == Y3Big::ROWS && Y2Big::TW == Y3Big::TW, "blk_gain: the 2-D and 3-D tiles cover the same positions");
    auto blk_gain = [&]() { return tile_efficiency<typename F::Y3Blk>(p.H, p.W) > 1.06 * tile_efficiency<Y3Big>(p.H, p.W); };
    if constexpr (BFV == 3) {
        if (k3 && p.vec4 && (tile_cfg == 6 || (auto_cfg && tile_workgroups<Y3Big>(d) >= 384 && tile_workgroups<typename F::Y3Blk>(d) >= 384 && blk_gain())))
            return launch_cfg<typename F::Y3Blk>(p, L);
        if (k2 && p.vec4 && p.Cout > 64 && (tile_cfg == 6 || (auto_cfg && tile_workgroups<Y2Big>(d) >= (scratch ? 96 : 384) && tile_workgroups<typename F::Y2Blk>(d) >= 384 && blk_gain())))
            return launch_cfg<typename F::Y2Blk>(p, L);
    }
    if (k3) {
        if (cfg == 0) cfg = tile_workgroups<Y3Big>(d) >= 384 ? 1 : (tile_workgroups<Y3Med>(d) >= (scratch ? 32 : 256) ? 2 : 3);
        if constexpr (BFV == 3) {
            const double e_b7 = tile_efficiency<typename F::Y3Blk7>(p.H, p.W), e_med = tile_efficiency<Y3Med>(p.H, p.W);
            if (p.vec4 && (tile_cfg == 7 || (auto_cfg && cfg == 2 && e_b7 > 1.06 * e_med)))
                return launch_cfg<typename F::Y3Blk7>(p, L);
        }
        if (cfg == 1) return launch_cfg<Y3Big>(p, L);
        if (cfg == 2) return launch_cfg<Y3Med>(p, L);
        return launch_cfg<Y3Small>(p, L);
    }
    if (k2) {
        if (p.Cout <= 64) return launch_cfg<Y2M64>(p, L);
        if (cfg == 0) {
            const int64_t need = scratch ? 96 : 384;
            cfg = tile_workgroups<Y2Big>(d) >= need ? 1 : (tile_workgroups<Y2Med>(d) >= need ? 2 : 3);
        }
        if (cfg == 1) return launch_cfg<Y2Big>(p, L);
        if (cfg == 2) return launch_cfg<Y2Med>(p, L);
        return launch_cfg<Y2Small>(p, L);
    }
    if (p.Cout <= 64) return launch_cfg<Y1M64>(p, L);
    if (tile_cfg == 3 && p.Cout % 256 == 0) return launch_cfg<Y1Wide>(p, L);
    if (auto_cfg && p.Cout % 256 == 0 && p.Cin >= p.Cout && !p.res && tile_workgroups<Y1Wide>(d) >= 128)
        return launch_cfg<Y1Wide>(p, L.without_scratch());
    if (cfg == 0 || cfg > 2) {
        if (BFV == 3) {
            cfg = 2;
        } else {
            cfg = (tile_workgroups<Y1Big>(d) >= (scratch ? 96 : 512)) ? 1 : 2;
            if (p.Cin <= 256 && p.Cout >= 4 * p.Cin && tile_workgroups<Y1Big>(d) < 2048) cfg = 2;
        }
    }
    if (cfg == 1) return launch_cfg<Y1Big>(p, L);
    return launch_cfg<Y1Small>(p, L);
}

}
```

### stem-seg_amd/csrc/encoder.hip

```cpp
#include "common.h"
#include <algorithm>
#include <cstddef>

namespace stemseg {

struct Padded2D {
    int64_t pitch, ts, cs, total, interior;
    Padded2D() = default;
    Padded2D(int C, int T, int H, int W) {
        pitch = round_up((int64_t)W + 2, 4);
        ts = (int64_t)(H + 2) * pitch;
        cs = (int64_t)T * ts;
        total = (int64_t)C * cs + 64;
        interior = pitch + 1;
    }
};
static inline StemsegVolume halo2d_view(float* base, int C, int T, int H, int W) {
    Padded2D g(C, T, H, W);
    return make_volume(base, g.cs, g.ts, g.pitch, C, T, H + 2, W + 2, g.total);
}
static inline StemsegVolume interior2d_view(float* base, int C, int T, int H, int W) {
    Padded2D g(C, T, H, W);
    return make_volume(base + g.interior, g.cs, g.ts, g.pitch, C, T, H, W, g.total - g.interior);
}
// ... 375 lines not shown
    const int64_t planes = (int64_t)fine.C * fine.T, f_ts = fine.t_stride, f_pitch = fine.y_stride;
    float* fine_halo = fine.ptr - (f_pitch + 1);
    const int own = up2_form(planes, H, W, f_ts, f_pitch, aligned16(fine_halo), fine_dense != nullptr, aligned16(fine_dense));
    if (fine_dense) {
        SS_CHECK_ARG(form == 0 || form == STEMSEG_UP2_FORM_DENSE, "upsample2x_add: form %d does not read a dense fine map", form);
        SS_CHECK_ARG(own == STEMSEG_UP2_FORM_DENSE,
                     "upsample2x_add: the dense form needs W %% 4 == 0 (W=%d), pitch %% 4 == 0, t_stride %% 4 == 0, 4 * %u groups <= pitch %lld, 16-byte aligned "
                     "haloed rows and dense map, and fewer than 2^32 items", W, up2_groups(W), (long long)f_pitch);
    } else {
        SS_CHECK_ARG(form != STEMSEG_UP2_FORM_DENSE, "upsample2x_add: the dense form needs a dense fine map");
        SS_CHECK_ARG(form != STEMSEG_UP2_FORM_VEC4X2 || own == STEMSEG_UP2_FORM_VEC4X2,
                     "upsample2x_add: the two-row form needs pitch %% 4 == 0, t_stride %% 4 == 0, 4 * %u groups <= pitch %lld, 16-byte aligned haloed rows and "
                     "fewer than 2^32 items", up2_groups(W), (long long)f_pitch);
    }
    const int used = form ? form : own;
    const unsigned gq = up2_groups(W);
    const int64_t items = planes * (H / 2 + 1) * gq;
    void* ev = profile_begin(50, 4.0 * (double)planes * (2.0 * H * W + (double)(H / 2) * (W / 2)), s);
    if (used == STEMSEG_UP2_FORM_DENSE)
        hipLaunchKernelGGL(upsample2x_add_dense_vec4x2_kernel, dim3((unsigned)ceil_div(items, 256)), dim3(256), 0, s, fine_halo, fine_dense,
                           (const float*)coarse.ptr, H, W, gq, (unsigned)items, f_ts, (int)f_pitch, coarse.t_stride, (int)coarse.y_stride);
    else if (used == STEMSEG_UP2_FORM_VEC4X2)
        hipLaunchKernelGGL(upsample2x_add_vec4x2_kernel, dim3((unsigned)ceil_div(items, 256)), dim3(256), 0, s, fine_halo, (const float*)coarse.ptr, H, W, gq,
                           (unsigned)items, f_ts, (int)f_pitch, coarse.t_stride, (int)coarse.y_stride);
    else
        hipLaunchKernelGGL(upsample2x_add_kernel, dim3(grid1d(planes * H * W)), dim3(256), 0, s, fine.ptr, (const float*)coarse.ptr, planes, H, W, f_ts, f_pitch,
                           coarse.t_stride, coarse.y_stride);
    profile_end(ev, s);
    SS_LAUNCH_CHECK();
    if (form_used) *form_used = used;
    return STEMSEG_OK;
}

static int launch_stem_s2d(const float* frames, int T, int H, int W, const StemsegVolume& v, hipStream_t s) {
    SS_CHECK_ARG(frames && v.ptr, "stem_s2d: null pointer");
    SS_CHECK_ARG(T >= 1 && H >= 2 && W >= 2 && H % 2 == 0 && W % 2 == 0, "stem_s2d: T=%d H=%d W=%d (H, W even)", T, H, W);
    SS_CHECK_ARG(reinterpret_cast<uintptr_t>(frames) % 8 == 0, "stem_s2d: frames must be 8-byte aligned");
    int rc = check_view("stem_s2d", "s2d", v);
    if (rc) return rc;
    SS_CHECK_ARG(v.C == 12 && v.T == T && v.H == H / 2 + 3 && v.W == W / 2 + 3 && v.c_stride == (int64_t)T * v.t_stride && v.y_stride < (1ll << 31),
                 "stem_s2d: the image must be [12][%d][%d][%d] with c_stride == T * t_stride, got [%d][%d][%d][%d]", T, H / 2 + 3, W / 2 + 3, v.C, v.T, v.H, v.W);
    hipLaunchKernelGGL(stem_s2d_kernel, dim3(grid1d((int64_t)T * 3 * H * (W / 2))), dim3(256), 0, s, frames, v.ptr, T, H, W, v.t_stride, (int)v.y_stride);
    SS_LAUNCH_CHECK();
    return STEMSEG_OK;
}

struct EncoderPlan {
    GuardList guards;
    int T, H, W, nblk[4], total_blocks;
    int h[4], w[4];
    int64_t V[4];
    int64_t S0, X1, A, B, Cst[4], M1[4], M2, DS, XS, L[4], FO[4], SK, SKfloats, total;
    int64_t LAT[3];
    int64_t S2D, s2d_ts, s2d_pitch;
    int groups, s3, mid[4];
    int64_t M1S[4];
    int plan_frames;
    int64_t plan_SKfloats;
};
constexpr int64_t ENC_PLAN_SK_FLOATS = 32ll << 20;

static int make_encoder_plan(const StemsegEncoderDesc* d, EncoderPlan& p) {
    SS_CHECK_ARG(d, "encoder: null descriptor");
    constexpr int32_t old_bytes = (int32_t)offsetof(StemsegEncoderDesc, conv2_groups);
    SS_CHECK_ARG(d->struct_bytes == (int32_t)sizeof(StemsegEncoderDesc) || d->struct_bytes == old_bytes,
                 "encoder: descriptor size mismatch (%d vs %d or %d): ABI skew", d->struct_bytes, (int)sizeof(StemsegEncoderDesc), (int)old_bytes);
    const bool has_arch = d->struct_bytes == (int32_t)sizeof(StemsegEncoderDesc);
    const int groups = has_arch && d->conv2_groups > 0 ? d->conv2_groups : 1;
    const int wpg = has_arch && d->width_per_group > 0 ? d->width_per_group : 64;
    SS_CHECK_ARG(!has_arch || (d->conv2_groups >= 0 && d->width_per_group >= 0 && (d->stride_in_3x3 == 0 || d->stride_in_3x3 == 1)),
                 "encoder: conv2_groups=%d width_per_group=%d stride_in_3x3=%d", d->conv2_groups, d->width_per_group, d->stride_in_3x3);
    if (groups == 1) {
        SS_CHECK_ARG(wpg == 64, "encoder: width_per_group=%d with one group (64 only)", wpg);
    } else {
        SS_CHECK_ARG((wpg == 4 || wpg == 8) && groups <= 1024 && (groups * wpg) % 32 == 0,
                     "encoder: %d groups x %d channels (width_per_group 4 or 8: 4..64 channels per group over the stages; groups x width a multiple of 32)",
                     groups, wpg);
    }
    p.groups = groups;
    p.s3 = has_arch ? d->stride_in_3x3 : 0;
    for (int i = 0; i < 4; ++i) p.mid[i] = (groups * wpg) << i;
    SS_CHECK_ARG(d->n_clips >= 1 && d->clip_frames >= 0 && d->clip_stride >= 0, "encoder: bad clip layout");
    if (d->clip_frames > 0) {
        SS_CHECK_ARG(d->clip_stride > 0 && (d->n_clips - 1) * d->clip_stride + d->clip_frames == d->T,
                     "encoder: %d windows of %d frames every %d frames do not cover T=%d", d->n_clips, d->clip_frames, d->clip_stride, d->T);
    } else {
        SS_CHECK_ARG(d->T % d->n_clips == 0, "encoder: T=%d is not n_clips=%d whole clips", d->T, d->n_clips);
    }
    SS_CHECK_ARG(d->T >= 1 && d->H >= 32 && d->W >= 32 && d->H % 32 == 0 && d->W % 32 == 0, "encoder: T=%d H=%d W=%d (H, W multiples of 32)", d->T, d->H, d->W);
    p.T = d->T; p.H = d->H; p.W = d->W;
    p.total_blocks = 0;
    for (int i = 0; i < 4; ++i) {
        SS_CHECK_ARG(d->blocks[i] >= 1 && d->blocks[i] <= 64, "encoder: blocks[%d]=%d", i, d->blocks[i]);
        p.nblk[i] = d->blocks[i];
        p.total_blocks += d->blocks[i];
        p.h[i] = d->H >> (2 + i); p.w[i] = d->W >> (2 + i);
        p.V[i] = (int64_t)d->T * p.h[i] * p.w[i];
    }
    SS_CHECK_ARG(p.total_blocks <= STEMSEG_MAX_ENCODER_BLOCKS, "encoder: more than %d bottleneck blocks", STEMSEG_MAX_ENCODER_BLOCKS);
    int64_t off = 0;
    p.guards.n = 0;
    auto take = [&](int64_t floats) {
        int64_t o = off;
        off += round_up(floats, 64);
        p.guards.push(off);
        off += WS_GUARD_FLOATS;
        return o;
    };
    p.S0 = take(64 * 4 * p.V[0]);
    p.s2d_pitch = round_up(d->W / 2 + 3, 4);
    p.s2d_ts = (int64_t)(d->H / 2 + 3) * p.s2d_pitch;
    p.S2D = take(12 * (int64_t)d->T * p.s2d_ts + 64);
    p.X1 = take(64 * p.V[0]);
    p.A = take(256 * p.V[0]);
    p.B = take(256 * p.V[0]);
    for (int i = 0; i < 4; ++i) {
        p.Cst[i] = take((int64_t)(256 << i) * p.V[i]);
        p.M1[i] = take(Padded2D(p.mid[i], p.T, p.h[i], p.w[i]).total);
    }
    p.M2 = take((int64_t)p.mid[0] * p.V[0]);
    p.DS = take(256 * p.V[0]);
    p.XS = take(256 * p.V[1]);
    for (int i = 0; i < 4; ++i) p.L[i] = take(Padded2D(256, p.T, p.h[i], p.w[i]).total);
    const bool shared_out = d->clip_frames > 0 && d->clip_stride < d->clip_frames && d->n_clips > 1;
    for (int i = 0; i < 4; ++i) p.FO[i] = shared_out ? take(256 * p.V[i]) : -1;
    for (int i = 0; i < 4; ++i) p.M1S[i] = (p.s3 && i > 0) ? take(Padded2D(p.mid[i], p.T, p.h[i - 1], p.w[i - 1]).total) : -1;
    SS_CHECK_ARG(d->plan_frames >= 0 && d->plan_frames <= 4096, "encoder: plan_frames=%d", d->plan_frames);
    p.plan_frames = d->plan_frames;
    p.plan_SKfloats = ENC_PLAN_SK_FLOATS;
    p.SKfloats = ENC_PLAN_SK_FLOATS * (d->plan_frames > 0 ? std::max<int64_t>(1, ceil_div(d->T, d->plan_frames)) : 1);
    p.SK = take(p.SKfloats);
    p.LAT[0] = p.S0;
    p.LAT[1] = p.X1;
    p.LAT[2] = take(256 * p.V[2]);
    p.total = off;
    SS_CHECK_ARG(!p.guards.full, "encoder: the plan has more than %d workspace slices (GuardList)", WS_MAX_GUARDS);
    return STEMSEG_OK;
}

static int run_stem(const EncoderPlan& p, const StemsegEncoderWeights* wts, int prec, const float* frames, float* s2d, float* stem_out, float* pooled,
                    hipStream_t s) {
    const int T = p.T;
    int rc;
    const int Ho = p.H / 2, Wo = p.W / 2;
    const int blocks = (int)(ceil_div(Wo, ST_COLS) * ceil_div(Ho, ST_ROWS) * T);
    void* ev = profile_begin(47, 4.0 * ((double)3 * T * p.H * p.W + 64.0 * T * Ho * Wo), s);
    if (wts->stem_w_s2d && prec == STEMSEG_PRECISION_F16X3 && p.W % 2 == 0) {
        const StemsegVolume in = make_volume(s2d, (int64_t)T * p.s2d_ts, p.s2d_ts, p.s2d_pitch, 12, T, Ho + 3, Wo + 3, 12 * (int64_t)T * p.s2d_ts + 64);
        rc = launch_stem_s2d(frames, T, p.H, p.W, in, s);
        if (rc) return rc;
        ConvEpilogue es;
        es.precision = prec;
        if (p.plan_frames > 0) { es.frames = T; es.plan_frames = p.plan_frames; es.plan_scratch_floats = p.plan_SKfloats; }
        es.relu = 1;
        rc = launch_conv3d(in, wts->stem_w_s2d, wts->stem_b, dense_volume(stem_out, 64, T, Ho, Wo), 1, 4, 4, 0, s, nullptr, 0, &es);
        if (rc) return rc;
    } else {
        hipLaunchKernelGGL(stem_conv7x7_mfma_kernel, dim3((unsigned)blocks), dim3(256), 0, s, frames, wts->stem_w, wts->stem_b, stem_out, T, p.H, p.W);
    }
    profile_end(ev, s);
    SS_LAUNCH_CHECK();
    return launch_maxpool3x3s2(stem_out, (int64_t)64 * T, Ho, Wo, pooled, 0, nullptr, s);
}

static int stage_end_mask(const StemsegEncoderDesc* d, const EncoderPlan& p) {
    int mask = 0;
    for (int k = 0; k < 3; ++k) {
        const int h = p.h[k], w = p.w[k], mid = p.mid[k];
        bool ok = ((d->fuse_tail >> k) & 1) && !((d->fuse_tail >> (6 + k)) & 1) && d->precision == STEMSEG_PRECISION_F16X3 && p.groups == 1 && !p.s3 &&
                  mid * 4 == (256 << k) && p.nblk[k] >= 2 && fused_stage_end_supported(mid, p.V[k]) && (int64_t)p.T * (h + 2) * (w + 4) <= (1ll << 27);
        Padded2D gf0(256, p.T, h, w);
// ... 118 lines not shown
    if (ws_bytes < (size_t)p.total * sizeof(float)) {
        set_error("encoder_stem_forward: workspace too small (%zu < %zu bytes)", ws_bytes, (size_t)p.total * sizeof(float));
        return STEMSEG_E_WORKSPACE;
    }
    SS_CHECK_ARG(wts->stem_w && wts->stem_b, "encoder_stem_forward: null stem weights");
    SS_CHECK_ARG(desc->precision == STEMSEG_PRECISION_F32 || desc->precision == STEMSEG_PRECISION_BF16X6 || desc->precision == STEMSEG_PRECISION_F16X3,
                 "encoder_stem_forward: precision must be 0 (f32), 2 (bf16x6) or 3 (f16x3)");
    return run_stem(p, wts, desc->precision, frames, reinterpret_cast<float*>(workspace) + p.S2D, stem_out, pooled, as_stream(stream));
}

extern "C" int stemseg_hip_encoder_forward(const StemsegEncoderDesc* desc, const StemsegEncoderWeights* wts, const float* frames,
                                           const StemsegVolume* out, void* workspace, size_t ws_bytes, void* stream) {
    EncoderPlan p;
    int rc = make_encoder_plan(desc, p);
    if (rc) return rc;
    SS_CHECK_ARG(wts && frames && out && workspace, "encoder_forward: null pointer");
    if (ws_bytes < (size_t)p.total * sizeof(float)) {
        set_error("encoder: workspace too small (%zu < %zu bytes)", ws_bytes, (size_t)p.total * sizeof(float));
        return STEMSEG_E_WORKSPACE;
    }
    SS_CHECK_ARG(wts->stem_w && wts->stem_b, "encoder_forward: null stem weights");
    for (int i = 0; i < 4; ++i) {
        for (int c = 0; c < desc->n_clips; ++c) {
            const StemsegVolume& o = out[4 * c + i];
            const int Tc_ = desc->clip_frames > 0 ? desc->clip_frames : p.T / desc->n_clips;
            SS_CHECK_ARG(o.ptr && o.C == desc->out_channels && o.T == Tc_ && o.H == p.h[i] && o.W == p.w[i],
                         "encoder_forward: output volume %d of clip %d must be [%d][%d][%d][%d]", i, c, desc->out_channels, Tc_, p.h[i], p.w[i]);
        }
        SS_CHECK_ARG(wts->fpn_inner_w[i] && wts->fpn_inner_b[i] && wts->fpn_layer_w[i] && wts->fpn_layer_b[i], "encoder_forward: null FPN weights %d", i);
    }
    SS_CHECK_ARG(desc->out_channels == 256, "encoder: out_channels must be 256");
    SS_CHECK_ARG(desc->precision == STEMSEG_PRECISION_F32 || desc->precision == STEMSEG_PRECISION_BF16X6 || desc->precision == STEMSEG_PRECISION_F16X3,
                 "encoder: precision must be 0 (f32), 2 (bf16x6) or 3 (f16x3)");
    const int prec = desc->precision;
    auto epi_for = [&](int frames) {
        ConvEpilogue e;
        e.precision = prec;
        if (p.plan_frames > 0) { e.frames = frames; e.plan_frames = p.plan_frames; e.plan_scratch_floats = p.plan_SKfloats; }
        return e;
    };
    hipStream_t s = as_stream(stream);
    float* ws = reinterpret_cast<float*>(workspace);
    const int T = p.T;

    rc = run_stem(p, wts, prec, frames, ws + p.S2D, ws + p.S0, ws + p.X1, s);
    if (rc) return rc;
    float* x = ws + p.X1;
    int cin = 64, bi = 0;
    bool conv1_done = false;
    const int end_mask = stage_end_mask(desc, p);
    bool lat_ok[3], end_done[3] = {false, false, false};
    for (int k = 0; k < 3; ++k)
        lat_ok[k] = ((end_mask >> k) & 1) && reinterpret_cast<uintptr_t>(ws + p.L[k]) % 16 == 0 && reinterpret_cast<uintptr_t>(ws + p.LAT[k]) % 16 == 0;
    for (int st = 0; st < 4; ++st) {
        const int mid = p.mid[st], cout = 256 << st, h = p.h[st], w = p.w[st];
        const int64_t V = p.V[st];
        for (int b = 0; b < p.nblk[st]; ++b, ++bi) {
            const bool first = (b == 0), stride2 = first && st > 0;
            const bool s3 = stride2 && p.s3;
            const bool grouped = p.groups > 1 || s3;
            SS_CHECK_ARG(wts->conv1_w[bi] && wts->conv1_b[bi] && wts->conv2_w[bi] && wts->conv2_b[bi] && wts->conv3_w[bi] && wts->conv3_b[bi],
                         "encoder_forward: null weights for block %d", bi);
            SS_CHECK_ARG(!first || (wts->down_w[bi] && wts->down_b[bi]), "encoder_forward: block %d needs a projection shortcut", bi);
            float* xin = x;
            if (stride2 && end_done[st - 1]) {
                xin = ws + p.XS;
            } else if (stride2) {
                rc = launch_encoder_subsample2(x, (int64_t)cin * T, 2 * h, 2 * w, ws + p.XS, 0, nullptr, s);
                if (rc) return rc;
                xin = ws + p.XS;
            }
            float* y = (b == p.nblk[st] - 1) ? ws + p.Cst[st] : ((b & 1) ? ws + p.B : ws + p.A);
            const int h1 = s3 ? 2 * h : h, w1 = s3 ? 2 * w : w;
            float* m1 = ws + (s3 ? p.M1S[st] : p.M1[st]);
            if (!conv1_done) {
                ConvEpilogue e1 = epi_for(T);
                e1.relu = 1; e1.dec_H = h1; e1.dec_W = w1;
                rc = launch_conv3d(flat_view(s3 ? x : xin, cin, (int64_t)T * h1 * w1), wts->conv1_w[bi], wts->conv1_b[bi], interior2d_view(m1, mid, T, h1, w1), 1, 1,
                                   1, 0, s, ws + p.SK, p.SKfloats, &e1);
                if (rc) return rc;
            }
            const bool want_fuse = ((desc->fuse_tail >> st) & 1) && prec == STEMSEG_PRECISION_F16X3 && b + 1 < p.nblk[st] && !grouped && p.groups == 1 &&
                                   mid * 4 == cout && fused_tail_supported(mid) && V <= (1ll << 27) && (int64_t)T * (h + 2) * (w + 4) <= (1ll << 27);
            const bool want_end = st < 3 && b + 1 == p.nblk[st] && lat_ok[st];
            int p16_done = 0;
            if (grouped) {
                rc = launch_grouped_conv(halo2d_view(m1, mid, T, h1, w1), wts->conv2_w[bi], wts->conv2_b[bi], dense_volume(ws + p.M2, mid, T, h, w), p.groups,
                                         s3 ? 2 : 1, 1, prec, s);
            } else {
                ConvEpilogue e2 = epi_for(T);
                e2.relu = 1;
                if (want_fuse) { e2.p16_out = reinterpret_cast<unsigned int*>(ws + p.M2); e2.p16_done = &p16_done; }
                if (want_end) { e2.p16_out = reinterpret_cast<unsigned int*>(ws + p.M2); e2.p16_done = &p16_done; e2.p16_keep_plan = 1; }
                rc = launch_conv3d(halo2d_view(m1, mid, T, h, w), wts->conv2_w[bi], wts->conv2_b[bi], dense_volume(ws + p.M2, mid, T, h, w), 1, 3, 3, 0, s,
                                   ws + p.SK, p.SKfloats, &e2);
            }
            if (rc) return rc;
            const float* idt = xin;
            ConvEpilogue ed = epi_for(T);
            const bool ds_in_tail = first && want_fuse && p16_done && !(desc->fuse_tail & 32) && st < 2 && !(st == 1 && ((desc->fuse_tail >> 3) & 3) == 1) &&
                                    fused_shortcut_supported(mid, cin, V);
            if (first && !ds_in_tail) {
                rc = launch_conv3d(flat_view(xin, cin, V), wts->down_w[bi], wts->down_b[bi], flat_view(ws + p.DS, cout, V), 1, 1, 1, 0, s, ws + p.SK, p.SKfloats,
                                   &ed);
                if (rc) return rc;
                idt = ws + p.DS;
            }
            if (want_fuse && p16_done) {
                SS_CHECK_ARG(wts->conv1_w[bi + 1] && wts->conv1_b[bi + 1], "encoder_forward: null weights for block %d", bi + 1);
                rc = launch_fused_tail(mid, reinterpret_cast<const unsigned int*>(ws + p.M2), wts->conv3_w[bi], wts->conv3_b[bi], ds_in_tail ? nullptr : idt, y,
                                       wts->conv1_w[bi + 1], wts->conv1_b[bi + 1], interior2d_view(ws + p.M1[st], mid, T, h, w), h, w, V, (desc->fuse_tail >> 3) & 3, s,
                                       ds_in_tail ? xin : nullptr, cin, ds_in_tail ? wts->down_w[bi] : nullptr, ds_in_tail ? wts->down_b[bi] : nullptr);
                if (rc) return rc;
                conv1_done = true;
            } else if (want_end && p16_done) {
                rc = launch_fused_stage_end(mid, reinterpret_cast<const unsigned int*>(ws + p.M2), wts->conv3_w[bi], wts->conv3_b[bi], idt, y, wts->fpn_inner_w[st],
                                            wts->fpn_inner_b[st], ws + p.LAT[st], ws + p.XS, T, h, w, s);
                if (rc) return rc;
                end_done[st] = true;
                conv1_done = false;
            } else {
                ConvEpilogue e3 = epi_for(T);
                e3.relu = 1; e3.res = idt; e3.res_cs = V; e3.res_ts = 0; e3.res_ys = 0;
                rc = launch_conv3d(flat_view(ws + p.M2, mid, V), wts->conv3_w[bi], wts->conv3_b[bi], flat_view(y, cout, V), 1, 1, 1, 0, s, ws + p.SK, p.SKfloats, &e3);
                if (rc) return rc;
                conv1_done = false;
            }
            x = y;
            cin = cout;
        }
    }
    for (int k = 3; k >= 0; --k) {
        const int h = p.h[k], w = p.w[k];
        ConvEpilogue e = epi_for(T), el = epi_for(T);
        e.dec_H = h; e.dec_W = w;
        Padded2D gf0(256, T, h, w);
        const bool lat_dense = k < 3 && up2_form((int64_t)256 * T, h, w, gf0.ts, gf0.pitch, aligned16(ws + p.L[k]), true, aligned16(ws + p.A)) == STEMSEG_UP2_FORM_DENSE;
        const bool lat_stored = k < 3 && end_done[k];
        const float* lat_map = lat_stored ? ws + p.LAT[k] : ws + p.A;
        if (lat_dense || lat_stored) {
            if (!lat_stored) {
                ConvEpilogue ed = epi_for(T);
                rc = launch_conv3d(flat_view(ws + p.Cst[k], 256 << k, p.V[k]), wts->fpn_inner_w[k], wts->fpn_inner_b[k], flat_view(ws + p.A, 256, p.V[k]), 1, 1, 1, 0, s,
                                   ws + p.SK, p.SKfloats, &ed);
                if (rc) return rc;
            }
            rc = launch_upsample2x_add(interior2d_view(ws + p.L[k], 256, T, h, w), lat_map, interior2d_view(ws + p.L[k + 1], 256, T, p.h[k + 1], p.w[k + 1]), 0,
                                       nullptr, s);
            if (rc) return rc;
        } else {
        rc = launch_conv3d(flat_view(ws + p.Cst[k], 256 << k, p.V[k]), wts->fpn_inner_w[k], wts->fpn_inner_b[k], interior2d_view(ws + p.L[k], 256, T, h, w), 1, 1, 1, 0, s,
                           ws + p.SK, p.SKfloats, &e);
        if (rc) return rc;
        }
        if (k < 3 && !lat_dense && !lat_stored) {
            rc = launch_upsample2x_add(interior2d_view(ws + p.L[k], 256, T, h, w), nullptr, interior2d_view(ws + p.L[k + 1], 256, T, p.h[k + 1], p.w[k + 1]), 0,
                                       nullptr, s);
            if (rc) return rc;
        }
        const int Tc = desc->clip_frames > 0 ? desc->clip_frames : T / desc->n_clips;
        const int Ts = desc->clip_frames > 0 ? desc->clip_stride : Tc;
        if (p.FO[k] >= 0) {
            rc = launch_conv3d(halo2d_view(ws + p.L[k], 256, T, h, w), wts->fpn_layer_w[k], wts->fpn_layer_b[k], dense_volume(ws + p.FO[k], 256, T, h, w), 1, 3, 3,
                               0, s, ws + p.SK, p.SKfloats, &el);
            if (rc) return rc;
            for (int c = 0; c < desc->n_clips; ++c) {
                rc = launch_copy_strided(ws + p.FO[k] + (int64_t)c * Ts * h * w, (int64_t)T * h * w, (int64_t)h * w, out[4 * c + k], s);
// ... 35 lines not shown
```

### stem-seg_amd/csrc/split_operand.h

```cpp
#pragma once
#include "common.h"

namespace stemseg {

constexpr float F16X3_ACT_SCALE = 0.25f;
constexpr float F16X3_LO_SCALE = 2048.0f;


__device__ __forceinline__ void split_pair_f16(const float x0, const float x1, unsigned int& hw, unsigned int& lw) {
    const float qs = F16X3_ACT_SCALE, ks = F16X3_LO_SCALE;
    unsigned int h, l;
    float r0, r1;
    asm("v_fma_mixlo_f16 %0, %1, %2, 0" : "=v"(h) : "v"(x0), "s"(qs));
    asm("v_fma_mixhi_f16 %0, %1, %2, 0" : "+v"(h) : "v"(x1), "s"(qs));
    asm("v_fma_mix_f32 %0, %1, %2, -%3 op_sel_hi:[0,0,1]" : "=v"(r0) : "v"(x0), "s"(qs), "v"(h));
    asm("v_fma_mix_f32 %0, %1, %2, -%3 op_sel:[0,0,1] op_sel_hi:[0,0,1]" : "=v"(r1) : "v"(x1), "s"(qs), "v"(h));
    asm("v_fma_mixlo_f16 %0, %1, %2, 0" : "=v"(l) : "v"(r0), "s"(ks));
    asm("v_fma_mixhi_f16 %0, %1, %2, 0" : "+v"(l) : "v"(r1), "s"(ks));
    hw = h;
    lw = l;
}

__device__ __forceinline__ void split_act_f16(const float x, unsigned short& hi, unsigned short& lo) {
    const float xs = x * F16X3_ACT_SCALE;
    const _Float16 fh = (_Float16)xs;
    const _Float16 fl = (_Float16)((xs - (float)fh) * F16X3_LO_SCALE);
    hi = __builtin_bit_cast(unsigned short, fh);
    lo = __builtin_bit_cast(unsigned short, fl);
}

__device__ __forceinline__ void split_bf16x3(const float x, __bf16& hi, __bf16& mid, __bf16& lo) {
    hi = (__bf16)x;
    const float r1 = x - (float)hi;
    mid = (__bf16)r1;
    lo = (__bf16)(r1 - (float)mid);
}
__device__ __forceinline__ void split_bf16x3(const float x, unsigned short& hi, unsigned short& mid, unsigned short& lo) {
    __bf16 bh, bm, bl;
    split_bf16x3(x, bh, bm, bl);
    hi = __builtin_bit_cast(unsigned short, bh);
    mid = __builtin_bit_cast(unsigned short, bm);
    lo = __builtin_bit_cast(unsigned short, bl);
}

__device__ __forceinline__ float f16x3_weight_scale(unsigned int max_bits) {
    const int e = (int)((max_bits >> 23) & 0xff);
    if (e == 0 || e == 0xff) return 1.0f;
    return __uint_as_float((unsigned int)min(max(127 + 13 - (e - 127), 1), 254) << 23);
}
__device__ __forceinline__ float f16x3_inv_scale(unsigned int max_bits) { return 1.0f / (f16x3_weight_scale(max_bits) * F16X3_ACT_SCALE); }

template <int PREC>
__device__ __forceinline__ unsigned short pack_split_weight(const float x, const int pl) {
    static_assert(PREC == STEMSEG_PRECISION_BF16X6 || PREC == STEMSEG_PRECISION_F16X3, "split-operand precisions");
    if constexpr (PREC == STEMSEG_PRECISION_F16X3) {
        const _Float16 hi = (_Float16)x;
        const _Float16 lo = (_Float16)(x - (float)hi);
        const _Float16 his = (_Float16)((float)hi * (1.0f / F16X3_LO_SCALE));
        return __builtin_bit_cast(unsigned short, pl == 0 ? hi : (pl == 1 ? lo : his));
    } else {
        __bf16 hi, mid, lo;
        split_bf16x3(x, hi, mid, lo);
        return __builtin_bit_cast(unsigned short, pl == 0 ? hi : (pl == 1 ? mid : lo));
    }
}


constexpr int split_chunk_channels(int taps, int prec) { return taps == 27 ? 4 : (taps == 9 ? (prec == STEMSEG_PRECISION_F16X3 ? 16 : 8) : (taps == 16 ? 16 : 32)); }

struct SplitLayout {
    int CK;
    int TPG;
    int CPH;
    int NTG, NCG;
    int G;
    int NPL;
    constexpr SplitLayout(int taps, int prec, int ck)
        : CK(ck), TPG(taps >= 27 ? 4 : ((taps >= 9 && ck < 16) ? 2 : 1)), CPH(8 / TPG), NTG((taps + TPG - 1) / TPG), NCG(ck / (2 * CPH)),
          G(NTG * NCG), NPL(prec == STEMSEG_PRECISION_BF16X6 ? 3 : 2) {}
    constexpr SplitLayout(int taps, int prec) : SplitLayout(taps, prec, split_chunk_channels(taps, prec)) {}
    constexpr int chunks(int Cin) const { return (Cin + CK - 1) / CK; }
    constexpr int chunk_pieces() const { return NPL * G * 2; }
    constexpr int64_t slab_bytes(int Cout, int Cin) const { return (int64_t)chunks(Cin) * chunk_pieces() * Cout * 16; }
    constexpr int64_t inv_offset(int Cout, int Cin) const { return slab_bytes(Cout, Cin); }
    constexpr int64_t max_bits_offset(int Cout, int Cin) const { return slab_bytes(Cout, Cin) + 4 * (int64_t)Cout; }
    constexpr int64_t bytes(int Cout, int Cin) const { return slab_bytes(Cout, Cin) + (NPL == 2 ? 8 * (int64_t)Cout : 0); }
};

}
```

### stem-seg_amd/stemseg_amd/hip.py

```python
import ctypes as C
import os

import torch

_HERE = os.path.dirname(os.path.abspath(__file__))
LIB_PATH = os.environ.get("STEMSEG_HIP_LIB") or os.path.join(_HERE, "lib", "libstemseg_hip.so")

MAX_INSTANCES = 64
MAX_EMB_DIMS = 8
ABI_VERSION = 11


class Volume(C.Structure):
    _fields_ = [("ptr", C.c_void_p), ("c_stride", C.c_int64), ("t_stride", C.c_int64), ("y_stride", C.c_int64),
                ("C", C.c_int32), ("T", C.c_int32), ("H", C.c_int32), ("W", C.c_int32), ("limit", C.c_int64)]


class DecoderDesc(C.Structure):
    _fields_ = [("struct_bytes", C.c_int32), ("in_channels", C.c_int32), ("inter", C.c_int32 * 4),
                ("T", C.c_int32), ("H4", C.c_int32), ("W4", C.c_int32), ("gn_groups", C.c_int32), ("gn_eps", C.c_float),
                ("pool", C.c_int32 * 3), ("t_scale", C.c_int32 * 3), ("n_out", C.c_int32),
                ("act", C.c_int32 * (2 * MAX_EMB_DIMS)), ("grid_axis", C.c_int32 * (2 * MAX_EMB_DIMS)),
                ("input_layout", C.c_int32), ("concurrency", C.c_int32), ("detached", C.c_int32), ("precision", C.c_int32),
                ("n_clips", C.c_int32), ("feat_clip_stride", C.c_int64 * 4), ("out_clip_stride", C.c_int64),
# ... 50 lines not shown
                ("seed_prob", C.c_float * MAX_INSTANCES)]


class ClusterItem(C.Structure):
    _fields_ = [("emb", C.c_void_p), ("bw", C.c_void_p), ("seed", C.c_void_p), ("n_max", C.c_int64), ("n_points_dev", C.c_void_p),
                ("label_start", C.c_int64), ("labels", C.c_void_p), ("meta_dev", C.c_void_p), ("opt_masks", C.c_void_p), ("opt_probs", C.c_void_p),
                ("workspace", C.c_void_p), ("ws_bytes", C.c_size_t)]


class EmbeddingLossDesc(C.Structure):
    _fields_ = [("struct_bytes", C.c_int32), ("embedding_size", C.c_int32), ("n_free_dims", C.c_int32), ("n_instances", C.c_int32),
                ("T", C.c_int32), ("H", C.c_int32), ("W", C.c_int32), ("reserved", C.c_int32), ("free_dim_bandwidths", C.c_float * MAX_EMB_DIMS)]


class TargetPrepDesc(C.Structure):
    _fields_ = [("struct_bytes", C.c_int32), ("n_instances", C.c_int32), ("T", C.c_int32), ("H", C.c_int32), ("W", C.c_int32),
                ("reserved", C.c_int32)]


class SemsegLossDesc(C.Structure):
    _fields_ = [("struct_bytes", C.c_int32), ("n_classes", C.c_int32), ("has_foreground_channel", C.c_int32), ("T", C.c_int32),
                ("H", C.c_int32), ("W", C.c_int32), ("reserved", C.c_int32), ("reserved2", C.c_int32), ("stride_c", C.c_int64),
                ("stride_t", C.c_int64), ("stride_h", C.c_int64), ("stride_w", C.c_int64)]


class OptTensor(C.Structure):
    _fields_ = [("p", C.c_void_p), ("g", C.c_void_p), ("state1", C.c_void_p), ("state2", C.c_void_p), ("n", C.c_int64), ("flags", C.c_int32),
                ("reserved", C.c_int32)]


class OptChunk(C.Structure):
    _fields_ = [("tensor", C.c_int32), ("chunk", C.c_int32)]


class OptHyper(C.Structure):
    _fields_ = [("struct_bytes", C.c_int32), ("flags", C.c_int32), ("lr", C.c_float), ("momentum", C.c_float), ("one_minus_dampening", C.c_float),
                ("weight_decay", C.c_float), ("one_minus_beta1", C.c_float), ("beta2", C.c_float), ("one_minus_beta2", C.c_float), ("eps", C.c_float)]


_P, _I32, _I64, _F = C.c_void_p, C.c_int32, C.c_int64, C.c_float
SIGNATURES = {
    "stemseg_hip_version": (C.c_int, []),
    "stemseg_hip_last_error": (C.c_char_p, []),
    "stemseg_hip_device_count": (C.c_int, []),
    "stemseg_hip_profile_enable": (C.c_int, [_I32]),
    "stemseg_hip_profile_read": (C.c_int, [C.POINTER(C.c_double), _I32]),
    "stemseg_hip_padded_geometry": (C.c_int, [_I32, _I32, _I32, _I32, C.POINTER(_I64)]),
    "stemseg_hip_pack_conv_weight": (C.c_int, [_P, _P, _I32, _I32, _I32, _P]),
    "stemseg_hip_encoder_plan_offsets": (C.c_int, [_P, _P]),
    "stemseg_hip_encoder_stage_end_mask": (C.c_int, [_P, C.POINTER(_I32)]),
    "stemseg_hip_packed_weight_bytes_prec": (C.c_int64, [_I32, _I32, _I32, _I32]),
    "stemseg_hip_pack_conv_weight_prec": (C.c_int, [_P, _P, _I32, _I32, _I32, _I32, _P]),
    "stemseg_hip_conv3d": (C.c_int, [C.POINTER(Volume), _P, _P, C.POINTER(Volume), _I32, _I32, _I32, _I32, _P, _I64, C.POINTER(ConvEpilogue), _P]),
    "stemseg_hip_packed_grouped_weight_bytes": (C.c_int64, [_I32, _I32, _I32, _I32]),
    "stemseg_hip_pack_grouped_conv_weight": (C.c_int, [_P, _P, _I32, _I32, _I32, _I32, _P]),
    "stemseg_hip_conv2d_grouped": (C.c_int, [C.POINTER(Volume), _P, _P, C.POINTER(Volume), _I32, _I32, _I32, _I32, _I32, _P]),
    "stemseg_hip_conv3d_gn_scratch_doubles": (C.c_int64, [_I32, _I32]),
    "stemseg_hip_conv3d_plan": (C.c_int, [C.POINTER(Volume), _P, C.POINTER(Volume), _I32, _I32, _I32, _I32, _P, _I64, C.POINTER(ConvEpilogue), _I32, _I32,
                                          C.POINTER(ConvPlanRecord), _I32, C.POINTER(_I32)]),
    "stemseg_hip_conv3d_plan_clips": (C.c_int, [C.POINTER(Volume), _P, C.POINTER(Volume), _I32, _I32, _I32, _I32, _P, _I64, C.POINTER(ConvEpilogue), _I32, _I32,
                                                _I32, C.POINTER(ConvPlanRecord), _I32, C.POINTER(_I32)]),
    "stemseg_hip_conv3d_zero_t_halo": (C.c_int, [C.POINTER(Volume), _P, _P, C.POINTER(Volume), _I32, _I32, _I32, _I32, _P, _I64, C.POINTER(ConvEpilogue),
                                                _I32, _F, _P, _P, _P]),
    "stemseg_hip_conv3d_zero_t_halo_clips": (C.c_int, [C.POINTER(Volume), _P, _P, C.POINTER(Volume), _I32, _I32, _I32, _I32, _P, _I64, C.POINTER(ConvEpilogue),
                                                      _I32, _F, _P, _P, _I32, _P]),
    "stemseg_hip_conv3d_zero_t_halo_batch": (C.c_int, [C.POINTER(Volume), _P, _P, C.POINTER(Volume), _I32, _I32, _I32, _I32, C.POINTER(ConvEpilogue),
                                                      _I32, _I64, _I64, _P]),
    "stemseg_hip_conv3d_gn": (C.c_int, [C.POINTER(Volume), _P, _P, C.POINTER(Volume), _I32, _I32, _I32, _I32, _P, _I64, _I32, _I32, _F, _P, _P, _P]),
    "stemseg_hip_stem_conv": (C.c_int, [_P, _P, _P, _P, _I32, _I32, _I32, _P]),
    "stemseg_hip_maxpool3x3s2": (C.c_int, [_P, _I64, _I32, _I32, _P, _I32, C.POINTER(_I32), _P]),
    "stemseg_hip_encoder_subsample2": (C.c_int, [_P, _I64, _I32, _I32, _P, _I32, C.POINTER(_I32), _P]),
    "stemseg_hip_upsample2x_add": (C.c_int, [C.POINTER(Volume), _P, C.POINTER(Volume), _I32, C.POINTER(_I32), _P]),
    "stemseg_hip_stem_s2d": (C.c_int, [_P, _I32, _I32, _I32, C.POINTER(Volume), _P]),
    "stemseg_hip_encoder_stream_forms": (C.c_int, [C.POINTER(EncoderDesc), C.POINTER(_I32)]),
    "stemseg_hip_encoder_workspace_bytes": (C.c_size_t, [C.POINTER(EncoderDesc)]),
    "stemseg_hip_encoder_init_workspace": (C.c_int, [C.POINTER(EncoderDesc), _P, C.c_size_t, _P]),
    "stemseg_hip_encoder_check_workspace": (C.c_int, [C.POINTER(EncoderDesc), _P, C.c_size_t, C.POINTER(_I32), C.POINTER(_I64), _P]),
    "stemseg_hip_encoder_forward": (C.c_int, [C.POINTER(EncoderDesc), C.POINTER(EncoderWeights), _P, C.POINTER(Volume), _P, C.c_size_t, _P]),
    "stemseg_hip_encoder_stem_forward": (C.c_int, [C.POINTER(EncoderDesc), C.POINTER(EncoderWeights), _P, _P, _P, _P, C.c_size_t, _P]),
    "stemseg_hip_groupnorm_stats": (C.c_int, [_P, _I32, _I64, _I32, _F, _P, _P, _P]),
    "stemseg_hip_gn_relu_pool": (C.c_int, [_P, _I32, _I32, _I32, _I32, _I32, _P, _P, _P, _I32, C.POINTER(Volume), _P]),
    "stemseg_hip_upsample_trilinear": (C.c_int, [_P, _I32, _I32, _I32, _I32, _I32, _I32, _I32, C.POINTER(Volume), _P]),
    "stemseg_hip_copy_to_volume": (C.c_int, [_P, _I32, C.POINTER(Volume), _P]),
    "stemseg_hip_heads": (C.c_int, [_P, _I32, _I32, _I32, _I32, _P, _P, _I32, C.POINTER(_I32), C.POINTER(_I32), _P, _P, _P, _P, _P]),
    "stemseg_hip_nonfinite_flags": (C.c_int, [_P, _I64, _P, _I32, _P]),
    "stemseg_hip_decoder_workspace_bytes": (C.c_size_t, [C.POINTER(DecoderDesc)]),
    "stemseg_hip_decoder_init_workspace": (C.c_int, [C.POINTER(DecoderDesc), _P, C.c_size_t, _P]),
    "stemseg_hip_decoder_check_workspace": (C.c_int, [C.POINTER(DecoderDesc), _P, C.c_size_t, C.POINTER(_I32), C.POINTER(_I64), _P]),
    "stemseg_hip_decoder_forward": (C.c_int, [C.POINTER(DecoderDesc), C.POINTER(DecoderWeights), C.POINTER(_P), _P, _P, C.c_size_t, _P]),
    "stemseg_hip_decoder_join": (C.c_int, [_I32, _P]),
    "stemseg_hip_seediness_accumulate": (C.c_int, [_P, _P, _I64, _I32, _P]),
    "stemseg_hip_fg_mask": (C.c_int, [_P, _F, _F, _P, _I64, _P]),
    "stemseg_hip_fg_mask_frames": (C.c_int, [_P, _P, _F, _P, _I32, _I64, _P]),
    "stemseg_hip_fg_gather": (C.c_int, [_P, _P, _P, _P, _I32, _I32, _I32, _I64, _P, _P, _P, _P, _P, _P, _P]),
    "stemseg_hip_cluster_workspace_bytes": (C.c_size_t, [_I64]),
    "stemseg_hip_cluster": (C.c_int, [_P, _P, _P, _I64, _P, _I32, _I32, C.POINTER(ClusterParams), _I64, _P, _P, _P, _P, _P, C.c_size_t, _P]),
    "stemseg_hip_cluster_batch": (C.c_int, [C.POINTER(ClusterItem), _I32, _I32, _I32, C.POINTER(ClusterParams), _P]),
    "stemseg_hip_overlap_counts": (C.c_int, [_P, _P, _I64, _P, _I32, _P, _I32, _I32, _I32, _P, _P, _P, _P]),
    "stemseg_hip_label_presence": (C.c_int, [_P, _I64, _P, _I32, _P, _I32, _P]),
    "stemseg_hip_relabel": (C.c_int, [_P, _I64, _P, _I32, _P]),
    "stemseg_hip_fg_compact": (C.c_int, [_P, _I32, _I64, _P, _P, _P, _P]),
    "stemseg_hip_labels_to_codes": (C.c_int, [_P, _P, _P, _I64, _I64, _P, _I64, _P]),
    "stemseg_hip_pair_tables": (C.c_int, [_P, _P, _P, _I32, _I64, _I32, _P, _P]),
    "stemseg_hip_codes_to_labels": (C.c_int, [_P, _P, _P, _I32, _I64, _P, _I64, _I32, _P, _P]),
    "stemseg_hip_semseg_accumulate": (C.c_int, [_P, _P, _I32, _I32, _I64, C.POINTER(C.c_int32), _I32, _P]),
    "stemseg_hip_semseg_masks": (C.c_int, [_P, _P, _I32, _I32, _I64, _I32, _P, _P, _P]),
# ... 294 lines not shown
    return list(out)


def _conv_epilogue(epilogue):
    if epilogue is None:
        return None
    e = ConvEpilogue()
    e.relu = int(epilogue.get("relu", 0))
    r = epilogue.get("residual")
    if r is not None:
        e.residual = r if isinstance(r, int) else r.data_ptr()
        e.res_c_stride, e.res_t_stride, e.res_y_stride = epilogue["res_strides"]
    e.decode_H, e.decode_W = epilogue.get("decode", (0, 0))
    e.precision = PRECISIONS[epilogue.get("precision", "f32")]
    e.frames, e.plan_frames, e.plan_scratch_floats = epilogue.get("plan", (0, 0, 0))
    return e


PLAN_GN, PLAN_ZERO_T_HALO = 1, 2
TILE_CFG_DEEP = 8
PLAN_REDUCE_FORMS = {0: None, 1: "vec16", 2: "scalar"}
PLAN_GN_FORMS = {0: None, 1: "tile epilogue", 2: "split-K reduce", 3: "separate pass"}


def conv3d_plan(vin, vout, k, tile_cfg=0, scratch=None, epilogue=None, bias=1 << 20, gn_groups=0, zero_t_halo=False, plan_clips=0):
    kt, kh, kw = (k, k, k) if isinstance(k, int) else k
    e = _conv_epilogue(epilogue)
    form = (PLAN_GN if gn_groups > 0 else 0) | (PLAN_ZERO_T_HALO if zero_t_halo else 0)
    addr, floats = scratch if scratch is not None else (None, 0)
    cap = 4
    rec, count = (ConvPlanRecord * cap)(), _I32(0)
    check(lib().stemseg_hip_conv3d_plan_clips(C.byref(vin), C.c_void_p(bias) if bias else None, C.byref(vout), kt, kh, kw, tile_cfg,
                                              C.c_void_p(addr) if addr else None, floats, C.byref(e) if e is not None else None, form, int(gn_groups),
                                              int(plan_clips), rec, cap, C.byref(count)))
    assert count.value <= cap, count.value
    out = []
    for r in rec[:count.value]:
        d = {n: getattr(r, n) for n, _ in ConvPlanRecord._fields_ if n != "grid"}
        d["grid"] = tuple(r.grid)
        d["precision"] = {v: n for n, v in PRECISIONS.items()}[r.precision]
        d["reduce"], d["gn"] = PLAN_REDUCE_FORMS[r.reduce], PLAN_GN_FORMS[r.gn]
        out.append(d)
    return out


def conv3d(vin, packed_w, bias, vout, k, tile_cfg=0, splitk_scratch=None, epilogue=None):
    n = 0 if splitk_scratch is None else splitk_scratch.numel()
    kt, kh, kw = (k, k, k) if isinstance(k, int) else k
    e = _conv_epilogue(epilogue)
    check(lib().stemseg_hip_conv3d(C.byref(vin), ptr(packed_w), ptr(bias), C.byref(vout), kt, kh, kw, tile_cfg,
                                   ptr(splitk_scratch), n, C.byref(e) if e is not None else None, stream()))


def conv3d_zero_t_halo(vin, packed_w, bias, vout, k=3, tile_cfg=0, splitk_scratch=None, precision="f32", gn_groups=0, eps=1e-5, plan_clips=0):
    n = 0 if splitk_scratch is None else splitk_scratch.numel()
    kt, kh, kw = (k, k, k) if isinstance(k, int) else k
    e = ConvEpilogue()
    e.precision = PRECISIONS[precision]
    stats = scratch = None
    if gn_groups > 0:
        stats = torch.empty(2 * gn_groups, dtype=torch.float32, device=packed_w.device)
        scratch = torch.empty(lib().stemseg_hip_conv3d_gn_scratch_doubles(vout.C, gn_groups), dtype=torch.float64, device=packed_w.device)
    check(lib().stemseg_hip_conv3d_zero_t_halo_clips(C.byref(vin), ptr(packed_w), ptr(bias), C.byref(vout), kt, kh, kw, tile_cfg, ptr(splitk_scratch), n,
                                                     C.byref(e), int(gn_groups), eps, ptr(stats), ptr(scratch), int(plan_clips), stream()))
    return stats


def conv3d_zero_t_halo_batch(vin, packed_w, bias, vout, n_clips, in_clip_stride, out_clip_stride, tile_cfg=0, precision="f32"):
    e = ConvEpilogue()
    e.precision = PRECISIONS[precision]
    check(lib().stemseg_hip_conv3d_zero_t_halo_batch(C.byref(vin), ptr(packed_w), ptr(bias), C.byref(vout), 3, 3, 3, tile_cfg, C.byref(e), int(n_clips),
                                                     int(in_clip_stride), int(out_clip_stride), stream()))


def conv3d_gn(vin, packed_w, bias, vout, k, groups, eps=1e-5, tile_cfg=0, splitk_scratch=None, precision="f32"):
    n = 0 if splitk_scratch is None else splitk_scratch.numel()
    kt, kh, kw = (k, k, k) if isinstance(k, int) else k
    dev = packed_w.device
    stats = torch.empty(2 * groups, dtype=torch.float32, device=dev)
    scratch = torch.empty(lib().stemseg_hip_conv3d_gn_scratch_doubles(vout.C, groups), dtype=torch.float64, device=dev)
    check(lib().stemseg_hip_conv3d_gn(C.byref(vin), ptr(packed_w), ptr(bias), C.byref(vout), kt, kh, kw, tile_cfg, ptr(splitk_scratch), n,
                                      PRECISIONS[precision], groups, eps, ptr(stats), ptr(scratch), stream()))
    return stats


def groupnorm_stats(x, groups, eps=1e-5):
    Cn = x.shape[0]
    S = x[0].numel()
    stats = torch.empty(2 * groups, dtype=torch.float32, device=x.device)
    scratch = torch.empty(groups * 128, dtype=torch.float64, device=x.device)
    check(lib().stemseg_hip_groupnorm_stats(ptr(x, torch.float32), Cn, S, groups, eps, ptr(stats), ptr(scratch), stream()))
    return stats


def gn_relu_pool(x, groups, stats, gamma, beta, pool, vout):
    Cn, T, H, W = x.shape
    check(lib().stemseg_hip_gn_relu_pool(ptr(x, torch.float32), Cn, T, H, W, groups, ptr(stats), ptr(gamma), ptr(beta),
                                         int(pool), C.byref(vout), stream()))


def upsample_trilinear(x, st, sy, sx, vout=None):
    Cn, T, H, W = x.shape
    out = None
    if vout is None:
        out = torch.empty(Cn, T * st, H * sy, W * sx, dtype=torch.float32, device=x.device)
        vout = dense_volume(out)
# ... 1552 lines not shown
```

Measured before the change: 128.7.

## Emit pre-split fp16 operand planes from fused tail into conv2 input

The fused bottleneck tail can now write the conv1 output directly as hi/lo fp16 operand planes in a haloed buffer. A new plane-input variant of the flat f16x3 1x3x3 conv tile reads those planes, so it no longer loads fp32 and splits it while staging. The encoder runs a probe conv per stage to check that the flat pmax-56 tile is the one selected, then routes conv2 through the plane path. The fp32 conv1 output is still written only for the last block. This adds a workspace buffer, a probe launch and a new kernel variant, and it is restricted to specific geometries.

```diff
diff --git a/include/stemseg_hip.h b/include/stemseg_hip.h
--- a/include/stemseg_hip.h
+++ b/include/stemseg_hip.h
@@ -71,6 +71,11 @@
 int stemseg_hip_conv3d_zero_t_halo_batch(const StemsegVolume* in, const float* packed_w, const float* bias, const StemsegVolume* out,
                                          int32_t kt, int32_t kh, int32_t kw, int32_t tile_cfg, const StemsegConvEpilogue* epilogue,
                                          int32_t n_clips, int64_t in_clip_stride, int64_t out_clip_stride, void* stream);
+
+int stemseg_hip_split_planes_haloed(const StemsegVolume* src, uint32_t* dst, void* stream);
+int stemseg_hip_conv2d_planes(const uint32_t* in_planes, const StemsegVolume* geometry, const float* packed_w, const float* bias,
+                              const StemsegVolume* out, int32_t tile_cfg, float* splitk_scratch, int64_t splitk_scratch_floats,
+                              const StemsegConvEpilogue* epilogue, uint32_t* out_planes, int32_t* out_planes_done, void* stream);
 
 typedef struct StemsegConvPlanRecord {
     int32_t kt, kh, kw;
diff --git a/stem-seg_amd/csrc/bottleneck_fused.hip b/stem-seg_amd/csrc/bottleneck_fused.hip
--- a/stem-seg_amd/csrc/bottleneck_fused.hip
+++ b/stem-seg_amd/csrc/bottleneck_fused.hip
@@ -24,6 +24,7 @@
     const float* bd;
     float* xsub;
     int sub_V;
+    unsigned int* z16;
 };
 
 constexpr SplitLayout FT_WL = SplitLayout(1, STEMSEG_PRECISION_F16X3);
@@ -375,6 +376,7 @@
         const int hwp = p.dec_H * p.dec_W;
         const int t2 = pos / hwp, r2 = pos - t2 * hwp, y2 = r2 / p.dec_W, x2 = r2 - y2 * p.dec_W;
         const unsigned int z_off = (unsigned int)(((int64_t)(4 * half) * p.z_cs + (int64_t)t2 * p.z_ts + (int64_t)y2 * p.z_ys + x2) * 4);
+        const unsigned int z16_off = (unsigned int)(((int64_t)t2 * p.z_ts + (int64_t)y2 * p.z_ys + x2) * 4 + 2 * half);
 #pragma unroll
         for (int m1 = 0; m1 < C::MI1; ++m1)
 #pragma unroll
@@ -382,11 +384,24 @@
                 const int co4 = m1 * 32 + 8 * q + 4 * half;
                 const float4 sc = *reinterpret_cast<const float4*>(reinterpret_cast<const float*>(xbuf) + co4);
                 const float4 bv = *reinterpret_cast<const float4*>(reinterpret_cast<const float*>(xbuf) + C::N1 + co4);
+                const float v0 = slot_act<C::LAT>(__fadd_rn(__fmul_rn(acc1[m1][4 * q + 0], sc.x), bv.x)), v1 = slot_act<C::LAT>(__fadd_rn(__fmul_rn(acc1[m1][4 * q + 1], sc.y), bv.y));
+                const float v2 = slot_act<C::LAT>(__fadd_rn(__fmul_rn(acc1[m1][4 * q + 2], sc.z), bv.z)), v3 = slot_act<C::LAT>(__fadd_rn(__fmul_rn(acc1[m1][4 * q + 3], sc.w), bv.w));
+                if constexpr (!C::LAT) {
+                    if (p.z16) {
+                        uint2 hw, lw;
+                        split_pair_f16(v0, v1, hw.x, lw.x);
+                        split_pair_f16(v2, v3, hw.y, lw.y);
+                        unsigned int* d = p.z16 + (int64_t)(m1 * 4 + q) * p.z_cs * 4 + z16_off;
+                        *reinterpret_cast<uint2*>(d) = hw;
+                        *reinterpret_cast<uint2*>(d + (int64_t)(C::N1 / 8) * p.z_cs * 4) = lw;
+                    }
+                    if (!p.z) continue;
+                }
                 char* zo = reinterpret_cast<char*>(p.z + (int64_t)(m1 * 32 + 8 * q) * p.z_cs);
-                *reinterpret_cast<float*>(zo + (size_t)z_off) = slot_act<C::LAT>(__fadd_rn(__fmul_rn(acc1[m1][4 * q + 0], sc.x), bv.x));
-                *reinterpret_cast<float*>(zo + p.z_cs * 4 + (size_t)z_off) = slot_act<C::LAT>(__fadd_rn(__fmul_rn(acc1[m1][4 * q + 1], sc.y), bv.y));
-                *reinterpret_cast<float*>(zo + p.z_cs * 8 + (size_t)z_off) = slot_act<C::LAT>(__fadd_rn(__fmul_rn(acc1[m1][4 * q + 2], sc.z), bv.z));
-                *reinterpret_cast<float*>(zo + p.z_cs * 12 + (size_t)z_off) = slot_act<C::LAT>(__fadd_rn(__fmul_rn(acc1[m1][4 * q + 3], sc.w), bv.w));
+                *reinterpret_cast<float*>(zo + (size_t)z_off) = v0;
+                *reinterpret_cast<float*>(zo + p.z_cs * 4 + (size_t)z_off) = v1;
+                *reinterpret_cast<float*>(zo + p.z_cs * 8 + (size_t)z_off) = v2;
+                *reinterpret_cast<float*>(zo + p.z_cs * 12 + (size_t)z_off) = v3;
             }
     }
 }
@@ -1017,6 +1032,7 @@
         const int hwp = p.dec_H * p.dec_W;
         const int t2 = pos / hwp, r2 = pos - t2 * hwp, y2 = r2 / p.dec_W, x2 = r2 - y2 * p.dec_W;
         const unsigned int z_off = (unsigned int)(((int64_t)(4 * half) * p.z_cs + (int64_t)t2 * p.z_ts + (int64_t)y2 * p.z_ys + x2) * 4);
+        const unsigned int z16_off = (unsigned int)(((int64_t)t2 * p.z_ts + (int64_t)y2 * p.z_ys + x2) * 4 + 2 * half);
         const float* ttab = reinterpret_cast<const float*>(w3buf);
 #pragma unroll
         for (int m1 = 0; m1 < C::MI1; ++m1)
@@ -1025,11 +1041,24 @@
                 const int co4 = m1 * 32 + 8 * q + 4 * half;
                 const float4 sc = *reinterpret_cast<const float4*>(ttab + co4);
                 const float4 bv = *reinterpret_cast<const float4*>(ttab + C::N1 + co4);
+                const float v0 = slot_act<C::LAT>(__fadd_rn(__fmul_rn(acc1[m1][4 * q + 0], sc.x), bv.x)), v1 = slot_act<C::LAT>(__fadd_rn(__fmul_rn(acc1[m1][4 * q + 1], sc.y), bv.y));
+                const float v2 = slot_act<C::LAT>(__fadd_rn(__fmul_rn(acc1[m1][4 * q + 2], sc.z), bv.z)), v3 = slot_act<C::LAT>(__fadd_rn(__fmul_rn(acc1[m1][4 * q + 3], sc.w), bv.w));
+                if constexpr (!C::LAT) {
+                    if (p.z16) {
+                        uint2 hw, lw;
+                        split_pair_f16(v0, v1, hw.x, lw.x);
+                        split_pair_f16(v2, v3, hw.y, lw.y);
+                        unsigned int* d = p.z16 + (int64_t)(m1 * 4 + q) * p.z_cs * 4 + z16_off;
+                        *reinterpret_cast<uint2*>(d) = hw;
+                        *reinterpret_cast<uint2*>(d + (int64_t)(C::N1 / 8) * p.z_cs * 4) = lw;
+                    }
+                    if (!p.z) continue;
+                }
                 char* zo = reinterpret_cast<char*>(p.z + (int64_t)(m1 * 32 + 8 * q) * p.z_cs);
-                *reinterpret_cast<float*>(zo + (size_t)z_off) = slot_act<C::LAT>(__fadd_rn(__fmul_rn(acc1[m1][4 * q + 0], sc.x), bv.x));
-                *reinterpret_cast<float*>(zo + p.z_cs * 4 + (size_t)z_off) = slot_act<C::LAT>(__fadd_rn(__fmul_rn(acc1[m1][4 * q + 1], sc.y), bv.y));
-                *reinterpret_cast<float*>(zo + p.z_cs * 8 + (size_t)z_off) = slot_act<C::LAT>(__fadd_rn(__fmul_rn(acc1[m1][4 * q + 2], sc.z), bv.z));
-                *reinterpret_cast<float*>(zo + p.z_cs * 12 + (size_t)z_off) = slot_act<C::LAT>(__fadd_rn(__fmul_rn(acc1[m1][4 * q + 3], sc.w), bv.w));
+                *reinterpret_cast<float*>(zo + (size_t)z_off) = v0;
+                *reinterpret_cast<float*>(zo + p.z_cs * 4 + (size_t)z_off) = v1;
+                *reinterpret_cast<float*>(zo + p.z_cs * 8 + (size_t)z_off) = v2;
+                *reinterpret_cast<float*>(zo + p.z_cs * 12 + (size_t)z_off) = v3;
             }
     }
 }
@@ -1099,16 +1128,24 @@
     p.V = (int)V;
     p.xs = nullptr; p.wd = nullptr; p.bd = nullptr;
     p.xsub = xsub; p.sub_V = (int)((int64_t)T * (h / 2) * (w / 2));
+    p.z16 = nullptr;
     if (mid == 256) { using C = FusedTailR1Cfg<256, 128, 0, 256, true>; return launch_stage_end_cfg<C>(fused_tail_r1_kernel<C>, p, s); }
     if (mid == 128) { using C = FusedTailR1Cfg<128, 128, 0, 256, true>; return launch_stage_end_cfg<C>(fused_tail_r1_kernel<C>, p, s); }
     using C = FusedTailCfg<64, 64, 128, 0, 256, true>;
     return launch_stage_end_cfg<C>(fused_tail_kernel<C>, p, s);
 }
 
+bool fused_tail_planes_supported(int mid, int64_t V, int form) {
+    return fused_tail_supported(mid) && !(mid == 256 && (form == 1 || (int64_t)128 * V * 4 >= (1ll << 32) - (1 << 20)));
+}
+
 int launch_fused_tail(int mid, const unsigned int* x16, const float* w3, const float* b3, const float* res, float* y, const float* w1, const float* b1,
                       const StemsegVolume& z, int dec_H, int dec_W, int64_t V, int form, hipStream_t s, const float* ds_x, int ds_cin, const float* ds_w,
-                      const float* ds_b) {
+                      const float* ds_b, unsigned int* z16, bool z_fp32) {
     SS_CHECK_ARG(x16 && w3 && b3 && y && w1 && b1 && z.ptr, "fused_tail: null pointer");
+    SS_CHECK_ARG(z_fp32 || z16, "fused_tail: the conv1 slot must write something");
+    SS_CHECK_ARG(!z16 || (reinterpret_cast<uintptr_t>(z16) % 8 == 0 && fused_tail_planes_supported(mid, V, form)),
+                 "fused_tail: operand planes need an 8-byte aligned slice and a 32-row-tile kernel (mid %d, form %d)", mid, form);
     SS_CHECK_ARG(ds_x ? (!res && ds_w && ds_b && fused_shortcut_supported(mid, ds_cin, V) && reinterpret_cast<uintptr_t>(ds_w) % 16 == 0 && reinterpret_cast<uintptr_t>(ds_b) % 16 == 0)
                       : res != nullptr, "fused_tail: identity map, or a shortcut (mid %d, %d input channels) this library has a kernel for", mid, ds_cin);
     SS_CHECK_ARG(fused_tail_supported(mid), "fused_tail: mid = %d (64, 128 or 256)", mid);
@@ -1124,6 +1161,8 @@
     p.V = (int)V;
     p.xs = ds_x; p.wd = reinterpret_cast<const char*>(ds_w); p.bd = ds_b;
     p.xsub = nullptr; p.sub_V = 0;
+    if (!z_fp32) p.z = nullptr;
+    p.z16 = z16;
     if (ds_x && mid == 128) return launch_fused_r1_cfg<FusedTailR1Cfg<128, 128, 256>>(p, s);
     if (ds_x) return launch_fused_cfg<FusedTailCfg<64, 128, 128, 64>>(p, s);
     if (mid == 256) {
diff --git a/stem-seg_amd/csrc/common.h b/stem-seg_amd/csrc/common.h
--- a/stem-seg_amd/csrc/common.h
+++ b/stem-seg_amd/csrc/common.h
@@ -129,6 +129,7 @@
     unsigned int* p16_out = nullptr;
     int* p16_done = nullptr;
     int p16_keep_plan = 0;
+    int in_planes = 0;
     int zero_t_halo = 0;
     PlanSink* plan_sink = nullptr;
 };
@@ -140,7 +141,8 @@
 bool fused_tail_supported(int mid);
 int launch_fused_tail(int mid, const unsigned int* x16, const float* w3, const float* b3, const float* res, float* y, const float* w1, const float* b1,
                       const StemsegVolume& z, int dec_H, int dec_W, int64_t V, int form, hipStream_t s, const float* ds_x = nullptr, int ds_cin = 0,
-                      const float* ds_w = nullptr, const float* ds_b = nullptr);
+                      const float* ds_w = nullptr, const float* ds_b = nullptr, unsigned int* z16 = nullptr, bool z_fp32 = true);
+bool fused_tail_planes_supported(int mid, int64_t V, int form);
 bool fused_shortcut_supported(int mid, int cin, int64_t V);
 int launch_gn_stats(const float* x, int C, int64_t S, int groups, float eps, float* stats, double* scratch, hipStream_t s);
 bool fused_stage_end_supported(int mid, int64_t V);
diff --git a/stem-seg_amd/csrc/conv_igemm.h b/stem-seg_amd/csrc/conv_igemm.h
--- a/stem-seg_amd/csrc/conv_igemm.h
+++ b/stem-seg_amd/csrc/conv_igemm.h
@@ -34,6 +34,7 @@
     int n_co;
     double* gn_part;
     int gn_cpg, gn_cap, gn_slot0;
+    int in_pln;
     int* gn_used_host;
     int nb;
     int zero_t_halo;
@@ -42,7 +43,7 @@
 };
 
 template <int KT_, int KH_, int KW_, int CK_, int MI_, int NI_, int WM_, int WN_, int COLS_, bool PIPE_ = false, int BF_ = 0, bool DB_ = false,
-          int PMAX_ = 0, bool GL_ = false, int BLK_ = 0>
+          int PMAX_ = 0, bool GL_ = false, int BLK_ = 0, bool PLN_ = false>
 struct ConvCfg {
     static constexpr bool PIPE = PIPE_, X6 = BF_ >= 2, F16 = BF_ == 3, DB = DB_, FLAT = PMAX_ > 0, GL = GL_;
     static_assert(BF_ == 0 || BF_ == 2 || BF_ == 3, "precision: 0 fp32-input MFMA, 2 bf16x6, 3 f16x3");
@@ -55,6 +56,7 @@
     static constexpr int MT = WM * MI * 32;
     static constexpr int NSEG = WN * NI;
     static constexpr bool BLK = BLK_ != 0;
+    static constexpr bool PLN = PLN_;
     static constexpr bool DEEP = BLK_ < 0;
     static constexpr int TD = DEEP ? WN_ : 1;
     static constexpr int TPL = DEEP ? TD + 2 : KT_;
@@ -90,6 +92,7 @@
     static_assert(LDS_FLOATS * 4 <= (X6 ? 160 : 80) * 1024, "two workgroups per CU (x6 eight-wave tiles: one)");
     static_assert(!X6 || (!DB && !GL && G >= 2 && CK % 2 == 0), "x6: 2-D / 3-D tiles, two weight phases");
     static_assert(!FLAT || (KH == 3 && KW == 3 && PMAX % 4 == 0), "flat tiles: 3x3 taps");
+    static_assert(!PLN_ || (BF_ == 3 && PMAX_ > 0 && KT_ == 1 && CK_ == 16 && SL.CPH == 8 && SL.TPG == 1 && SL.NCG == 1), "plane input: the flat f16x3 1x3x3 tile, a k-group = one tap x two octets");
     static_assert(DB == GL_, "two LDS buffers are the direct-to-LDS form");
     static_assert(!GL || (DB && !X6), "direct-to-LDS staging is the double-buffered fp32 form");
     static constexpr int NWAVES = WM * WN;
@@ -169,11 +172,12 @@
 #pragma unroll
     for (int ni = 0; ni < C::NI; ++ni) {
         const int s = wn * C::NI + ni;
-        b_ptr6[ni] = C::FLAT ? reinterpret_cast<const unsigned int*>(in_lds) + half * (C::CPH / 2) * C::IN_PAIR_STRIDE + s * 32 + l31 + 3
+        b_ptr6[ni] = C::PLN  ? reinterpret_cast<const unsigned int*>(in_lds) + (half * C::FL + s * 32 + l31 + 3) * 4
+                   : C::FLAT ? reinterpret_cast<const unsigned int*>(in_lds) + half * (C::CPH / 2) * C::IN_PAIR_STRIDE + s * 32 + l31 + 3
                              : reinterpret_cast<const unsigned int*>(in_lds) + half * (C::CPH / 2) * C::IN_PAIR_STRIDE + seg_row(min(s, C::NLIVE - 1), l31) * C::XP + seg_col(min(s, C::NLIVE - 1), l31);
         if constexpr (C::DEEP) b_ptr6[ni] += wn * (C::RH * C::XP);
     }
-    const float* in_tile = p.in + (int64_t)blockIdx.y * p.in_bs + (int64_t)t * p.in_ts + x0;
+    const float* in_tile = p.in + (int64_t)blockIdx.y * p.in_bs + (int64_t)t * p.in_ts * (C::PLN ? 4 : 1) + x0;
     const int64_t tile_base = (int64_t)t * p.in_ts + x0;
 
     constexpr int XQ = C::XP / 4;
@@ -335,7 +339,23 @@
     constexpr int NQ6V = TV ? (C::CK / 2) * 2 * R6 : NQ6;
     constexpr int IN_PT6V = TV ? (NQ6V + C::NTHREADS - 1) / C::NTHREADS : IN_PT6;
     auto in6_live = [](const int qv, const int first) __attribute__((always_inline)) { return qv + (qv / (2 * R6)) * R6 + (first ? R6 : 0); };
-    if constexpr (C::X6) {
+    auto pln_rel = [&](const int q, int& oct) __attribute__((always_inline)) -> int64_t {
+        oct = q / C::FL;
+        const int j = q % C::FL, f = F0 - pitch - 4 + j;
+        if (f < 0 || j >= C::NT + 2 * pitch + 8 || (int64_t)t * p.in_ts + f >= p.in_cs) return -1;
+        return ((int64_t)oct * p.in_cs + f) * 4;
+    };
+    const int64_t pln_plane_bytes = (int64_t)(p.Cin / 2) * p.in_cs * 4;
+    if constexpr (C::PLN) {
+#pragma unroll
+        for (int k = 0; k < IN_PT6; ++k) {
+            const int q = tid + k * C::NTHREADS;
+            int oct = 0;
+            const int64_t rel = q < NQ6 ? pln_rel(q, oct) : -1;
+            in6_voff[k] = rel < 0 ? 0u : (unsigned int)(rel * 4);
+            in6_clim[k] = rel < 0 ? 0 : p.Cin - 8 * oct;
+        }
+    } else if constexpr (C::X6) {
 #pragma unroll
         for (int k = 0; k < IN_PT6; ++k) {
             int q = tid + k * C::NTHREADS;
@@ -354,7 +374,13 @@
     }
     typedef float f32x4 __attribute__((ext_vector_type(4)));
     auto fetch_in6_fast = [&](int c0, int k, f32x4& v0, f32x4& v1) __attribute__((always_inline)) {
-        const char* base = reinterpret_cast<const char*>(in_tile) + (int64_t)c0 * p.in_cs * 4;
+        const char* base = reinterpret_cast<const char*>(in_tile) + (int64_t)c0 * p.in_cs * (C::PLN ? 2 : 4);
+        if constexpr (C::PLN) {
+            const unsigned int off = c0 < in6_clim[k] ? in6_voff[k] : 0u;
+            v0 = *reinterpret_cast<const f32x4*>(base + off);
+            v1 = *reinterpret_cast<const f32x4*>(base + pln_plane_bytes + off);
+            return;
+        }
         const unsigned int cs4 = (unsigned int)(p.in_cs * 4);
         v0 = *reinterpret_cast<const f32x4*>(base + (c0 < in6_clim[k] ? in6_voff[k] : 0u));
         v1 = *reinterpret_cast<const f32x4*>(base + (c0 + 1 < in6_clim[k] ? in6_voff[k] + cs4 : 0u));
@@ -380,6 +406,13 @@
         if constexpr (C::NPX == 3) *reinterpret_cast<uint4*>(d + 2 * C::IN_PLANE_STRIDE) = pl;
     };
     auto store_in6_masked = [&](int c0, int k, int q, const f32x4& r0, const f32x4& r1) __attribute__((always_inline)) {
+        if constexpr (C::PLN) {
+            const bool ok = c0 < in6_clim[k];
+            const f32x4 z = {0.f, 0.f, 0.f, 0.f};
+            *reinterpret_cast<f32x4*>(in_lds + q * 4) = ok ? r0 : z;
+            *reinterpret_cast<f32x4*>(in_lds + q * 4 + C::IN_PLANE_STRIDE) = ok ? r1 : z;
+            return;
+        }
         const bool ok0 = c0 < in6_clim[k], ok1 = c0 + 1 < in6_clim[k];
         float4 v0, v1;
         v0.x = ok0 ? r0.x : 0.f; v0.y = ok0 ? r0.y : 0.f; v0.z = ok0 ? r0.z : 0.f; v0.w = ok0 ? r0.w : 0.f;
@@ -387,7 +420,20 @@
         store_in6(q, v0, v1);
     };
     auto stage_in6_direct = [&](int c0) {
-        if (p.vec4) {
+        if constexpr (C::PLN) {
+            const char* base = reinterpret_cast<const char*>(in_tile) + (int64_t)c0 * p.in_cs * 2;
+            for (int q = tid; q < NQ6; q += C::NTHREADS) {
+                int oct;
+                const int64_t rel = pln_rel(q, oct);
+                f32x4 v0 = {0.f, 0.f, 0.f, 0.f}, v1 = v0;
+                if (rel >= 0 && c0 + 8 * oct < p.Cin) {
+                    v0 = *reinterpret_cast<const f32x4*>(base + rel * 4);
+                    v1 = *reinterpret_cast<const f32x4*>(base + pln_plane_bytes + rel * 4);
+                }
+                *reinterpret_cast<f32x4*>(in_lds + q * 4) = v0;
+                *reinterpret_cast<f32x4*>(in_lds + q * 4 + C::IN_PLANE_STRIDE) = v1;
+            }
+        } else if (p.vec4) {
             for (int q = tid; q < NQ6; q += C::NTHREADS) {
                 float4 v0, v1;
                 fetch_in6(c0, q, v0, v1);
@@ -435,7 +481,7 @@
         const unsigned int* bdy6[C::NI][3];
         if constexpr (C::FLAT) {
 #pragma unroll
-            for (int ni = 0; ni < C::NI; ++ni) { bdy6[ni][0] = b_ptr6[ni]; bdy6[ni][1] = b_ptr6[ni] + pitch; bdy6[ni][2] = b_ptr6[ni] + 2 * pitch; }
+            for (int ni = 0; ni < C::NI; ++ni) { bdy6[ni][0] = b_ptr6[ni]; bdy6[ni][1] = b_ptr6[ni] + pitch * (C::PLN ? 4 : 1); bdy6[ni][2] = b_ptr6[ni] + 2 * pitch * (C::PLN ? 4 : 1); }
         }
         auto ld_b = [&](const int grp, h16x8 (&b)[NPX][C::NI]) __attribute__((always_inline)) {
             const int cg = grp / C::NTG, tg = grp % C::NTG;
@@ -443,6 +489,11 @@
             for (int ni = 0; ni < (LIVE1 ? C::NI : 1); ++ni)
 #pragma unroll
                 for (int pl = 0; pl < NPX; ++pl) {
+                    if constexpr (C::PLN) {
+                        const int dy = (grp / C::KW) % C::KH, dx = grp % C::KW;
+                        b[pl][ni] = *reinterpret_cast<const h16x8*>(bdy6[ni][dy] + pl * C::IN_PLANE_STRIDE + dx * 4);
+                        continue;
+                    }
                     uint4 w4;
                     unsigned int* wv = reinterpret_cast<unsigned int*>(&w4);
 #pragma unroll
diff --git a/stem-seg_amd/csrc/conv_igemm.hip b/stem-seg_amd/csrc/conv_igemm.hip
--- a/stem-seg_amd/csrc/conv_igemm.hip
+++ b/stem-seg_amd/csrc/conv_igemm.hip
@@ -142,6 +142,13 @@
         p.out_p16 = epi->p16_out;
         p.gn_used_host = epi->p16_done;
     }
+    p.in_pln = 0;
+    if (epi && epi->in_planes) {
+        SS_CHECK_ARG(k2 && prec == STEMSEG_PRECISION_F16X3 && in.C % 8 == 0 && epi->nb <= 1 && reinterpret_cast<uintptr_t>(in.ptr) % 16 == 0 &&
+                     in.c_stride == (int64_t)in.T * in.t_stride && in.limit >= (int64_t)in.C * in.c_stride && in.c_stride < (1ll << 26),
+                     "conv3d: a plane-form input needs f16x3, 1x3x3 taps, whole channel octets, c_stride == T * t_stride and no clip batch");
+        p.in_pln = 1;
+    }
     p.nb = (epi && epi->nb > 1) ? epi->nb : 1;
     p.in_bs = p.nb > 1 ? epi->in_bs : 0; p.out_bs = p.nb > 1 ? epi->out_bs : 0; p.gn_bs = p.nb > 1 ? epi->gn_bs : 0;
     SS_CHECK_ARG(p.nb == 1 || (!p.res && p.nb <= 65535 && p.in_bs % 4 == 0 && p.out_bs % 4 == 0), "conv3d: a clip batch takes no residual and 16-byte aligned clip strides");
@@ -383,3 +390,52 @@
                                              StemsegConvPlanRecord* records, int32_t capacity, int32_t* count) {
     return conv3d_plan(in, bias, out, kt, kh, kw, tile_cfg, splitk_scratch, splitk_scratch_floats, epilogue, form, gn_groups, plan_clips, records, capacity, count);
 }
+
+namespace stemseg {
+
+__global__ __launch_bounds__(256) void split_planes_haloed_kernel(const float* __restrict__ src, unsigned int* __restrict__ dst, int64_t S, int64_t n) {
+    const int64_t i = (int64_t)blockIdx.x * 256 + threadIdx.x;
+    if (i >= n) return;
+    const int64_t o = i / S, pos = i - o * S;
+    const float* s = src + o * 8 * S + pos;
+    uint4 hw, lw;
+    split_pair_f16(s[0], s[S], hw.x, lw.x);
+    split_pair_f16(s[2 * S], s[3 * S], hw.y, lw.y);
+    split_pair_f16(s[4 * S], s[5 * S], hw.z, lw.z);
+    split_pair_f16(s[6 * S], s[7 * S], hw.w, lw.w);
+    *reinterpret_cast<uint4*>(dst + i * 4) = hw;
+    *reinterpret_cast<uint4*>(dst + (n + i) * 4) = lw;
+}
+
+}
+
+extern "C" int stemseg_hip_split_planes_haloed(const StemsegVolume* src, uint32_t* dst, void* stream) {
+    using namespace stemseg;
+    SS_CHECK_ARG(src && src->ptr && dst, "split_planes_haloed: null pointer");
+    int rc = check_view("split_planes_haloed", "src", *src);
+    if (rc) return rc;
+    SS_CHECK_ARG(src->C % 8 == 0 && src->c_stride == (int64_t)src->T * src->t_stride && src->limit >= (int64_t)src->C * src->c_stride &&
+                 reinterpret_cast<uintptr_t>(dst) % 16 == 0,
+                 "split_planes_haloed: the haloed view of [C][T][H + 2][pitch] with C %% 8 == 0 and c_stride == T * t_stride; dst 16-byte aligned");
+    const int64_t n = (int64_t)(src->C / 8) * src->c_stride;
+    SS_CHECK_ARG(n > 0 && ceil_div(n, 256) < (1ll << 31), "split_planes_haloed: volume too large");
+    hipLaunchKernelGGL(split_planes_haloed_kernel, dim3((unsigned)ceil_div(n, 256)), dim3(256), 0, as_stream(stream), (const float*)src->ptr, dst, src->c_stride, n);
+    SS_LAUNCH_CHECK();
+    return STEMSEG_OK;
+}
+
+extern "C" int stemseg_hip_conv2d_planes(const uint32_t* in_planes, const StemsegVolume* geometry, const float* packed_w, const float* bias,
+                                         const StemsegVolume* out, int32_t tile_cfg, float* splitk_scratch, int64_t splitk_scratch_floats,
+                                         const StemsegConvEpilogue* epilogue, uint32_t* out_planes, int32_t* out_planes_done, void* stream) {
+    using namespace stemseg;
+    SS_CHECK_ARG(in_planes && geometry && out, "conv2d_planes: null pointer");
+    ConvEpilogue e = epilogue_from_abi(epilogue);
+    e.in_planes = 1;
+    int done = 0;
+    if (out_planes) { e.p16_out = out_planes; e.p16_done = &done; }
+    StemsegVolume in = *geometry;
+    in.ptr = reinterpret_cast<float*>(const_cast<uint32_t*>(in_planes));
+    const int rc = launch_conv3d(in, packed_w, bias, *out, 1, 3, 3, tile_cfg, as_stream(stream), splitk_scratch, splitk_scratch_floats, &e);
+    if (out_planes_done) *out_planes_done = done;
+    return rc;
+}
diff --git a/stem-seg_amd/csrc/conv_split_family.h b/stem-seg_amd/csrc/conv_split_family.h
--- a/stem-seg_amd/csrc/conv_split_family.h
+++ b/stem-seg_amd/csrc/conv_split_family.h
@@ -22,6 +22,10 @@
     using Y3Blk = ConvCfg<3, 3, 3, 4, 4, 2, 1, 8, 3, false, BFV, false, 0, false, 5>;
     using Y2Blk = ConvCfg<1, 3, 3, CK2, 4, 2, 1, 8, 3, false, BFV, false, 0, false, 5>;
     using Y3Blk7 = ConvCfg<3, 3, 3, 4, 2, 2, 2, 4, 7, false, BFV, false, 0, false, 1>;
+};
+
+struct PlaneTiles {
+    using Y2FlatPln56 = ConvCfg<1, 3, 3, 16, 4, 2, 1, 8, 16, false, 3, false, 56, false, 0, true>;
 };
 
 struct DeepTiles {
@@ -52,12 +56,15 @@
             const double efl = (double)d.T * p.H * p.W / (512.0 * ceil_div((int64_t)d.T * p.in_ts, 512));
             if (tile_cfg == 5 || (efl > 1.04 * e2d && p.in_ys <= 56)) {
                 p.flat_t = 1;
+                if (p.in_ys <= 56 && p.in_pln) return launch_cfg<PlaneTiles::Y2FlatPln56>(p, L);
+                SS_CHECK_ARG(!p.in_pln, "conv3d: no plane-input form of the flat tile at row pitch %lld (<= 56)", (long long)p.in_ys);
                 if (p.in_ys <= 56) return launch_cfg<typename F::template Y2Flat<56>>(p, L);
                 if (p.in_ys <= 112) return launch_cfg<typename F::template Y2Flat<112>>(p, L);
                 return launch_cfg<typename F::template Y2Flat<224>>(p, L);
             }
         }
     }
+    SS_CHECK_ARG(!p.in_pln, "conv3d: this launch takes a tile without a plane-input form (the flat f16x3 1x3x3 tile at row pitch <= 56 has one)");
     if constexpr (BFV == 3) {
         if (deep_tile_eligible<DeepTiles::Y3Deep>(p, d, L, k3)) return launch_cfg<DeepTiles::Y3Deep>(p, L);
     }
diff --git a/stem-seg_amd/csrc/encoder.hip b/stem-seg_amd/csrc/encoder.hip
--- a/stem-seg_amd/csrc/encoder.hip
+++ b/stem-seg_amd/csrc/encoder.hip
@@ -451,6 +451,7 @@
     int64_t V[4];
     int64_t S0, X1, A, B, Cst[4], M1[4], M2, DS, XS, L[4], FO[4], SK, SKfloats, total;
     int64_t LAT[3];
+    int64_t M1P[3];
     int64_t S2D, s2d_ts, s2d_pitch;
     int groups, s3, mid[4];
     int64_t M1S[4];
@@ -516,6 +517,10 @@
     for (int i = 0; i < 4; ++i) {
         p.Cst[i] = take((int64_t)(256 << i) * p.V[i]);
         p.M1[i] = take(Padded2D(p.mid[i], p.T, p.h[i], p.w[i]).total);
+        if (i < 3) {
+            const Padded2D g(p.mid[i], p.T, p.h[i], p.w[i]);
+            p.M1P[i] = (g.pitch <= 56 && groups == 1 && !p.s3) ? take(g.total) : -1;
+        }
     }
     p.M2 = take((int64_t)p.mid[0] * p.V[0]);
     p.DS = take(256 * p.V[0]);
@@ -740,9 +745,22 @@
     bool lat_ok[3], end_done[3] = {false, false, false};
     for (int k = 0; k < 3; ++k)
         lat_ok[k] = ((end_mask >> k) & 1) && reinterpret_cast<uintptr_t>(ws + p.L[k]) % 16 == 0 && reinterpret_cast<uintptr_t>(ws + p.LAT[k]) % 16 == 0;
+    bool conv1_planes = false;
     for (int st = 0; st < 4; ++st) {
         const int mid = p.mid[st], cout = 256 << st, h = p.h[st], w = p.w[st];
         const int64_t V = p.V[st];
+        bool pln_stage = false;
+        if (st < 3 && p.M1P[st] >= 0 && prec == STEMSEG_PRECISION_F16X3 && !(desc->fuse_tail & 512) && ((desc->fuse_tail >> st) & 1) && p.groups == 1 && !p.s3 && mid % 16 == 0 &&
+            p.nblk[st] >= 2 && wts->conv2_w[bi] && fused_tail_planes_supported(mid, V, (desc->fuse_tail >> 3) & 3)) {
+            StemsegConvPlanRecord rec[2];
+            PlanSink sink{rec, 2, 0};
+            ConvEpilogue ep = epi_for(T);
+            ep.relu = 1; ep.plan_sink = &sink;
+            rc = launch_conv3d(halo2d_view(ws + p.M1[st], mid, T, h, w), wts->conv2_w[bi], wts->conv2_b[bi], dense_volume(ws + p.M2, mid, T, h, w), 1, 3, 3, 0, s,
+                               ws + p.SK, p.SKfloats, &ep);
+            if (rc) return rc;
+            pln_stage = sink.n == 1 && rec[0].flat == 1 && rec[0].pmax == 56 && rec[0].precision == STEMSEG_PRECISION_F16X3;
+        }
         for (int b = 0; b < p.nblk[st]; ++b, ++bi) {
             const bool first = (b == 0), stride2 = first && st > 0;
             const bool s3 = stride2 && p.s3;
@@ -780,8 +798,9 @@
                 e2.relu = 1;
                 if (want_fuse) { e2.p16_out = reinterpret_cast<unsigned int*>(ws + p.M2); e2.p16_done = &p16_done; }
                 if (want_end) { e2.p16_out = reinterpret_cast<unsigned int*>(ws + p.M2); e2.p16_done = &p16_done; e2.p16_keep_plan = 1; }
-                rc = launch_conv3d(halo2d_view(m1, mid, T, h, w), wts->conv2_w[bi], wts->conv2_b[bi], dense_volume(ws + p.M2, mid, T, h, w), 1, 3, 3, 0, s,
-                                   ws + p.SK, p.SKfloats, &e2);
+                if (conv1_done && conv1_planes) e2.in_planes = 1;
+                rc = launch_conv3d(halo2d_view(e2.in_planes ? ws + p.M1P[st] : m1, mid, T, h, w), wts->conv2_w[bi], wts->conv2_b[bi], dense_volume(ws + p.M2, mid, T, h, w), 1,
+                                   3, 3, 0, s, ws + p.SK, p.SKfloats, &e2);
             }
             if (rc) return rc;
             const float* idt = xin;
@@ -798,9 +817,12 @@
                 SS_CHECK_ARG(wts->conv1_w[bi + 1] && wts->conv1_b[bi + 1], "encoder_forward: null weights for block %d", bi + 1);
                 rc = launch_fused_tail(mid, reinterpret_cast<const unsigned int*>(ws + p.M2), wts->conv3_w[bi], wts->conv3_b[bi], ds_in_tail ? nullptr : idt, y,
                                        wts->conv1_w[bi + 1], wts->conv1_b[bi + 1], interior2d_view(ws + p.M1[st], mid, T, h, w), h, w, V, (desc->fuse_tail >> 3) & 3, s,
-                                       ds_in_tail ? xin : nullptr, cin, ds_in_tail ? wts->down_w[bi] : nullptr, ds_in_tail ? wts->down_b[bi] : nullptr);
+                                       ds_in_tail ? xin : nullptr, cin, ds_in_tail ? wts->down_w[bi] : nullptr, ds_in_tail ? wts->down_b[bi] : nullptr,
+                                       pln_stage ? reinterpret_cast<unsigned int*>(ws + p.M1P[st]) + Padded2D(mid, T, h, w).interior * 4 : nullptr,
+                                       !pln_stage || b + 2 == p.nblk[st]);
                 if (rc) return rc;
                 conv1_done = true;
+                conv1_planes = pln_stage;
             } else if (want_end && p16_done) {
                 rc = launch_fused_stage_end(mid, reinterpret_cast<const unsigned int*>(ws + p.M2), wts->conv3_w[bi], wts->conv3_b[bi], idt, y, wts->fpn_inner_w[st],
                                             wts->fpn_inner_b[st], ws + p.LAT[st], ws + p.XS, T, h, w, s);
diff --git a/stem-seg_amd/csrc/split_operand.h b/stem-seg_amd/csrc/split_operand.h
--- a/stem-seg_amd/csrc/split_operand.h
+++ b/stem-seg_amd/csrc/split_operand.h
@@ -66,6 +66,7 @@
 }
 
 
+
 constexpr int split_chunk_channels(int taps, int prec) { return taps == 27 ? 4 : (taps == 9 ? (prec == STEMSEG_PRECISION_F16X3 ? 16 : 8) : (taps == 16 ? 16 : 32)); }
 
 struct SplitLayout {
diff --git a/stem-seg_amd/stemseg_amd/hip.py b/stem-seg_amd/stemseg_amd/hip.py
--- a/stem-seg_amd/stemseg_amd/hip.py
+++ b/stem-seg_amd/stemseg_amd/hip.py
@@ -126,6 +126,8 @@
     "stemseg_hip_packed_weight_bytes_prec": (C.c_int64, [_I32, _I32, _I32, _I32]),
     "stemseg_hip_pack_conv_weight_prec": (C.c_int, [_P, _P, _I32, _I32, _I32, _I32, _P]),
     "stemseg_hip_conv3d": (C.c_int, [C.POINTER(Volume), _P, _P, C.POINTER(Volume), _I32, _I32, _I32, _I32, _P, _I64, C.POINTER(ConvEpilogue), _P]),
+    "stemseg_hip_split_planes_haloed": (C.c_int, [C.POINTER(Volume), _P, _P]),
+    "stemseg_hip_conv2d_planes": (C.c_int, [_P, C.POINTER(Volume), _P, _P, C.POINTER(Volume), _I32, _P, _I64, C.POINTER(ConvEpilogue), _P, C.POINTER(_I32), _P]),
     "stemseg_hip_packed_grouped_weight_bytes": (C.c_int64, [_I32, _I32, _I32, _I32]),
     "stemseg_hip_pack_grouped_conv_weight": (C.c_int, [_P, _P, _I32, _I32, _I32, _I32, _P]),
     "stemseg_hip_conv2d_grouped": (C.c_int, [C.POINTER(Volume), _P, _P, C.POINTER(Volume), _I32, _I32, _I32, _I32, _I32, _P]),
@@ -526,6 +528,21 @@
                                    ptr(splitk_scratch), n, C.byref(e) if e is not None else None, stream()))
 
 
+def split_planes_haloed(vsrc):
+    out = torch.empty(vsrc.C * vsrc.c_stride, dtype=torch.int32, device="cuda")
+    check(lib().stemseg_hip_split_planes_haloed(C.byref(vsrc), ptr(out), stream()))
+    return out
+
+
+def conv2d_planes(planes, vgeom, packed_w, bias, vout, tile_cfg=0, splitk_scratch=None, epilogue=None, out_planes=None):
+    n = 0 if splitk_scratch is None else splitk_scratch.numel()
+    e = _conv_epilogue(epilogue if epilogue is not None else dict(precision="f16x3"))
+    done = _I32(0)
+    check(lib().stemseg_hip_conv2d_planes(ptr(planes), C.byref(vgeom), ptr(packed_w), ptr(bias), C.byref(vout), tile_cfg, ptr(splitk_scratch), n,
+                                          C.byref(e), ptr(out_planes), C.byref(done), stream()))
+    return bool(done.value)
+
+
 def conv3d_zero_t_halo(vin, packed_w, bias, vout, k=3, tile_cfg=0, splitk_scratch=None, precision="f32", gn_groups=0, eps=1e-5, plan_clips=0):
     n = 0 if splitk_scratch is None else splitk_scratch.numel()
     kt, kh, kw = (k, k, k) if isinstance(k, int) else k
```

After: 128.9 (median of 6 runs). No clear change (+0.2%).
